# vwxyzjn/cleanrl

Measured on NVIDIA H100. Metric: env steps/sec (SPS) PPO Breakout num_envs=1024, higher is better.
Workload: dtype bf16

## Files before the change

### cleanrl_b200/csrc/net_tc.cu

```cuda
#include <cuda.h>
#include <algorithm>
#include "tc_base.cuh"
#include "tc_conv_win.cuh"
#include "tc_conv1_u8.cuh"
#include "tc_gemm_tma.cuh"
#include "tc_wgrad_win.cuh"
#include "tc_reduce.cuh"
#include "tc_aux.cuh"
#include "tc_heads.cuh"
#include "tc_heads_wide.cuh"
#include "tc_lstm.cuh"

namespace b200rl {

struct NatureLayout {
    int A;
    int64_t c1w, c1b, c2w, c2b, c3w, c3b, fcw, fcb, hw, hb, total;
    int64_t w1f, w2f, w2dg, w3f, w3dg, wfcf, wfcdg, w1l, w1sc, packed_total;
    bool wide; int G; int64_t whf, whdg, hbp;
    int64_t wih, whh, bih, bhh, whhp;
    explicit NatureLayout(int A_) : A(A_), wih(-1), whh(-1), bih(-1), bhh(-1), whhp(-1) {
        int64_t o = 0;
        c1w = o; o += 32 * 4 * 8 * 8;  c1b = o; o += 32;
        c2w = o; o += 64 * 32 * 4 * 4; c2b = o; o += 64;
        c3w = o; o += 64 * 64 * 3 * 3; c3b = o; o += 64;
        fcw = o; o += 512 * 3136;      fcb = o; o += 512;
        hw = o;  o += (int64_t)(A + 1) * 512;
        hb = o;  o += A + 1;
        total = o;
        int64_t q = 0;
        w1f = q; q += 32 * 256;
        w2f = q; q += 64 * 512;
        w2dg = q; q += 4 * 32 * 256;
        w3f = q; q += 64 * 576;
        w3dg = q; q += 64 * 576;
        wfcf = q; q += 512 * 3136;
        wfcdg = q; q += 3136 * 512;
        w1l = q; q += 64 * 256 / 2;
        w1sc = q; q += 64 * 2;
        wide = A + 1 > kMaxHeads;
        G = wide ? (int)ceil_div(A + 1, kWideHeadPad) * kWideHeadPad : 0;
        whf = whdg = hbp = 0;
        if (wide) {
            whf = q; q += (int64_t)G * 512;
            whdg = q; q += (int64_t)G * 512;
            hbp = q; q += (int64_t)G * 2;
        }
        packed_total = q;
    }
    struct Lstm {};
    NatureLayout(int A_, Lstm) : A(A_) {
        int64_t o = 0;
        c1w = o; o += 32 * 8 * 8;      c1b = o; o += 32;
        c2w = o; o += 64 * 32 * 4 * 4; c2b = o; o += 64;
        c3w = o; o += 64 * 64 * 3 * 3; c3b = o; o += 64;
        fcw = o; o += 512 * 3136;      fcb = o; o += 512;
        wih = o; o += 512 * 512;       whh = o; o += 512 * 128;
        bih = o; o += 512;             bhh = o; o += 512;
        hw = o;  o += (int64_t)(A + 1) * 128;
        hb = o;  o += A + 1;
        total = o;
        int64_t q = 0;
        w1f = q; q += 32 * 64;
        w2f = q; q += 64 * 512;
        w2dg = q; q += 4 * 32 * 256;
        w3f = q; q += 64 * 576;
        w3dg = q; q += 64 * 576;
        wfcf = q; q += 512 * 3136;
        wfcdg = q; q += 3136 * 512;
        w1l = w1sc = -1;
        wide = true; G = 512;
        whf = q; q += 512 * 512;
        whdg = q; q += 512 * 512;
        hbp = q; q += 512 * 2;
        whhp = q; q += 512 * 128;
        packed_total = q;
    }
};

struct NatureActs {
    int64_t x0, act1, act2, act3, hid, dhid, dact3a, dact3b, dact2a, dact2b, dact1, m1, m2, m3, m4, total;
    explicit NatureActs(int64_t n, bool with_x0 = true) {
        int64_t o = 0;
        x0 = o; if (with_x0) o += n * 28224;
        act1 = o; o += n * 12800;
        act2 = o; o += n * 5184;
        act3 = o; o += n * 3136;
        hid = o;  o += n * 512;
        dhid = o; o += n * 512;
        dact3a = o; o += n * 5184;
        dact3b = o; o += n * 7744;
        dact2a = o; o += n * 6400;
        dact2b = o; o += n * 7744;
        dact1 = o; o += n * 14112;
        auto pad8 = [](int64_t v) { return (v + 7) & ~int64_t(7); };
        m1 = o; o += pad8(n * 100 * 4 * 2);
        m2 = o; o += pad8(n * 81 * 2 * 2);
        m3 = o; o += pad8(n * 49 * 2 * 2);
        m4 = o; o += pad8(n * 16 * 2);
        total = o;
    }
};

static void gemm_rowmajor(KGemmParams& p, const bf16* x, int64_t n, int nchunks) {
    memset(&p, 0, sizeof(p));
    p.scale = 1.f;
    p.A = x; p.M = n; p.nchunks = nchunks;
}


static void win_defaults(WinParams& p) { memset(&p, 0, sizeof(p)); p.scale = 1.f; }
static int round8(int v) { return (v + 7) & ~7; }
static void win_conv1(WinParams& p, const bf16* x0, const int64_t* rows, int64_t n) {
    p.A = x0; p.rows = rows; p.n = (int)n; p.G = 441; p.Wp = 21; p.M = n * 441;
    p.tpi_shift = 2;
    p.n_images = rows ? (int64_t)1 << 24 : n;
    p.ntaps = 4; p.shift[0] = 0; p.shift[1] = 1; p.shift[2] = 21; p.shift[3] = 22; p.WR = round8(128 + 22);
}
static void win_conv2(WinParams& p, const bf16* act1, int64_t n) {
    p.A = act1; p.n = (int)n; p.G = 100; p.Wp = 10; p.M = n * 100;
    p.ntaps = 4; p.shift[0] = 0; p.shift[1] = 1; p.shift[2] = 10; p.shift[3] = 11; p.WR = round8(128 + 11);
}
static void win_conv3(WinParams& p, const bf16* act2, int64_t n) {
    p.A = act2; p.n = (int)n; p.G = 81; p.Wp = 9; p.M = n * 81;
    p.ntaps = 9; for (int ky = 0; ky < 3; ++ky) for (int kx = 0; kx < 3; ++kx) p.shift[ky * 3 + kx] = ky * 9 + kx;
    p.WR = round8(128 + 20);
}
static void wgw_defaults(WGradWinParams& w) { memset(&w, 0, sizeof(w)); }

static const int kC1Ctas = 264, kC2Ctas = 132, kC3Ctas = 132;
static WPlan conv1_wgrad_plan(int64_t n, bool u8) {
    return u8 ? wgrad_plan(n * 512, kC2Ctas, 512) : wgrad_plan(n * 512, kC1Ctas, 128);
}
static WPlan conv2_wgrad_plan(int64_t n) { return wgrad_plan(n * 100, kC2Ctas, 128); }
static WPlan conv3_wgrad_plan(int64_t n) { return wgrad_plan(n * 81, kC3Ctas, 128); }

static size_t wgrad_win_bytes(int splits, int nslots) { return (size_t)splits * nslots * 64 * 64 * sizeof(float); }
static size_t wgrad_win_bias_bytes(int splits) { return (size_t)splits * 64 * sizeof(float); }
static int launch_wgrad_win(const WGradWinParams& p, int ctas, cudaStream_t s, const char* what) {
    const size_t smem = (size_t)kWgradWinStages * ((size_t)p.WRX * 128 * p.cpr + 128 * 128) + 4096 + 1024;
    static SmemAttrCache attr;
    if (int rc0 = attr.ensure(tc_wgrad_win, smem, what)) return rc0;
    CUtensorMap tmX, tmY;
    memset(&tmX, 0, sizeof(tmX)); memset(&tmY, 0, sizeof(tmY));
    const int use_tma = p.tpi_shift ? 0 : 1;
    if (p.rows_per_cta % 128 != 0) return fail(B200RL_ERR_INVALID_ARGUMENT, "%s: rows per CTA must be a multiple of 128", what);
    if (ctas < 1 || (int64_t)(ctas - 1) * p.rows_per_cta >= p.M)
        return fail(B200RL_ERR_INVALID_ARGUMENT, "%s: every row split must own at least one row", what);
    int rc;
    if (use_tma) {
        if (p.rows || p.ldy != 64 || p.ncolsY != 64)
            return fail(B200RL_ERR_INVALID_ARGUMENT, "%s: linear-grid mode needs contiguous rows and 64-channel dY", what);
        if ((rc = make_tmap_2d(&tmX, p.X, p.M, (int64_t)p.cpr * 64, p.WRX, what))) return rc;
        if ((rc = make_tmap_2d(&tmY, p.Y, p.M, 64, 128, what))) return rc;
    } else {
        if ((128 << p.tpi_shift) < p.G) return fail(B200RL_ERR_INVALID_ARGUMENT, "%s: steps per image too small", what);
        if ((rc = make_tmap_3d(&tmX, p.X, p.n_images, p.G, (int64_t)p.cpr * 64, p.WRX, what))) return rc;
    }
    const dim3 grid((unsigned)ceil_div(p.nslots / 2, kWgradWinTilesPerCta), ctas);
    tc_wgrad_win<<<grid, kWgradWinThreads, smem, s>>>(tmX, tmY, p, use_tma);
    return check_launch(what);
}

}

using namespace b200rl;

namespace b200rl {
static bool head_ok(int A) { return A >= 1 && A < kMaxWideHeads; }
static size_t wide_dhead_bytes(int64_t n, const NatureLayout& L) { return ((size_t)n * L.G * 2 + 255) & ~(size_t)255; }
static size_t wide_small_bytes(int64_t n, const NatureLayout& L, int A1) {
    return wide_dhead_bytes(n, L) + colsum_f32_ws(n, A1);
}

static int trunk_fwd(const NatureLayout& L, const NatureActs& Q, const float* params, const bf16* P, bf16* act, int64_t n,
                     cudaStream_t s) {
    int rc;
    KGemmParams p;
    WinParams wp;
    win_defaults(wp); win_conv2(wp, act + Q.act1, n);
    wp.Bw = P + L.w2f; wp.N = 64; wp.vH = 9; wp.vW = 9; wp.out_mode = WOUT_DENSE; wp.out = act + Q.act2;
    wp.bias = params + L.c2b; wp.relu = 1; wp.mask_out = reinterpret_cast<uint32_t*>(act + Q.m2);
    { ProfScope ps(s, "conv2_fwd", 2.0 * n * 81 * 64 * 512, (double)n * ((12800 + 5184) * 2 + 648));
      if ((rc = launch_conv_win_t<128, 2, 2, 4>(wp, s, "naturecnn/conv2"))) return rc; }
    win_defaults(wp); win_conv3(wp, act + Q.act2, n);
    wp.Bw = P + L.w3f; wp.N = 64; wp.vH = 7; wp.vW = 7; wp.out_mode = WOUT_DENSE; wp.out = act + Q.act3;
    wp.bias = params + L.c3b; wp.relu = 1; wp.mask_out = reinterpret_cast<uint32_t*>(act + Q.m3);
    { ProfScope ps(s, "conv3_fwd", 2.0 * n * 49 * 64 * 576, (double)n * ((5184 + 3136) * 2 + 392));
      if ((rc = launch_conv_win_t<128, 1, 4, 9>(wp, s, "naturecnn/conv3"))) return rc; }
    gemm_rowmajor(p, act + Q.act3, n, 49);
    p.Bw = P + L.wfcf; p.N = 512; p.out = act + Q.hid; p.ldo = 512; p.bias = params + L.fcb; p.relu = 1;
    p.mask_out = reinterpret_cast<uint32_t*>(act + Q.m4);
    { ProfScope ps(s, "fc_fwd", 2.0 * n * 512 * 3136, (double)n * (3136 + 512) * 2 + 512.0 * 3136 * 2);
      if (n <= 8192) { if ((rc = launch_gemm_tma<64, 6>(p, s, "naturecnn/fc"))) return rc; }
      else if ((rc = launch_gemm_tma<128, 4>(p, s, "naturecnn/fc"))) return rc; }
    return B200RL_OK;
}

static int trunk_bwd(const NatureLayout& L, const NatureActs& Q, const bf16* P, bf16* act, float* grads, int64_t n,
                     float* wsbig, float* wssmall, void* tail_ready_event, bool dact1_fused, cudaStream_t s) {
    int rc;
    KGemmParams p;
    {
        int splits;
        { ProfScope ps(s, "fc_wgrad", 2.0 * n * 512 * 3136, (double)n * (3136 + 512) * 2 + 512.0 * 3136 * 4);
          if ((splits = launch_wgrad_tma(act + Q.dhid, 512, act + Q.act3, 3136, n, wsbig, s, "naturecnn/fc_wgrad")) < 0) return splits; }
        { ProfScope ps(s, "wgrad_fold_bias", 0, 0);
          note_launches(1); tc_fold_fc<<<(unsigned)ceil_div((int64_t)512 * 3136, 256), 256, 0, s>>>(wsbig, splits, 512, 13 * 256, 512, 3136, 64, 49, 1.f, grads + L.fcw);
          if ((rc = colsum(act + Q.dhid, n, 512, 512, wssmall, grads + L.fcb, s))) return rc; }
        if (tail_ready_event) {
            cudaError_t e = cudaEventRecord(reinterpret_cast<cudaEvent_t>(tail_ready_event), s);
            if (e != cudaSuccess) return fail(B200RL_ERR_CUDA, "naturecnn_backward: cudaEventRecord: %s", cudaGetErrorString(e));
        }
        gemm_rowmajor(p, act + Q.dhid, n, 8);
        p.Bw = P + L.wfcdg; p.N = 3136; p.out = act + Q.dact3a; p.out2 = act + Q.dact3b; p.dual_dact3 = 1;
        p.ldo = 3136; p.mask_bits = reinterpret_cast<const uint32_t*>(act + Q.m3);
        { ProfScope ps(s, "fc_dgrad", 2.0 * n * 512 * 3136, (double)n * ((3136 + 512) * 2 + 392) + 512.0 * 3136 * 2);
          if ((rc = launch_gemm_tma<128, 4>(p, s, "naturecnn/fc_dgrad"))) return rc; }
    }
    WGradWinParams gw;
    WinParams wp;
    FoldWin fw;
    {
        wgw_defaults(gw);
        gw.X = act + Q.act2; gw.M = n * 81; gw.n = (int)n; gw.G = 81; gw.cpr = 1; gw.nslots = 10; gw.WRX = round8(128 + 20);
        for (int t = 0; t < 9; ++t) gw.shift[t] = (t / 3) * 9 + (t % 3);
        const int st[10] = {0, 1, 2, 3, 4, 5, 6, 7, 7, 8};
        for (int k = 0; k < 10; ++k) { gw.slot_tap[k] = st[k]; gw.slot_cc[k] = 0; }
        gw.Y = act + Q.dact3a; gw.ldy = 64; gw.ncolsY = 64;
        const WPlan pl = conv3_wgrad_plan(n);
        gw.rows_per_cta = pl.rows_per_cta; gw.ws = wsbig; gw.wsb = wssmall;
        { ProfScope ps(s, "conv3_wgrad", 2.0 * n * 49 * 64 * 576, (double)n * (5184 + 5184) * 2);
          if ((rc = launch_wgrad_win(gw, pl.splits, s, "naturecnn/conv3_wgrad"))) return rc; }
        memset(&fw, 0, sizeof(fw));
        fw.layer = 3; fw.S = pl.splits; fw.nslots = 10; fw.Cout = 64; fw.scale = 1.f; fw.bscale = 1.f;
        for (int k = 0; k < 10; ++k) { fw.slot_tap[k] = st[k]; fw.slot_skip[k] = (k == 8); }
        { ProfScope ps(s, "wgrad_fold_bias", 0, 0);
          fw.wsb = wssmall; fw.db = grads + L.c3b;
          tc_fold_win<<<(unsigned)ceil_div(640 * 64 + 64, 32), 256, 0, s>>>(wsbig, fw, grads + L.c3w);
          if ((rc = check_launch("naturecnn/conv3_fold"))) return rc; }
        win_defaults(wp);
        wp.A = act + Q.dact3b; wp.n = (int)n; wp.G = 121; wp.Wp = 11; wp.M = n * 121; wp.ntaps = 9;
        for (int ky = 0; ky < 3; ++ky) for (int kx = 0; kx < 3; ++kx) wp.shift[ky * 3 + kx] = (2 - ky) * 11 + (2 - kx);
        wp.WR = round8(128 + 24);
        wp.Bw = P + L.w3dg; wp.N = 64; wp.vH = 9; wp.vW = 9; wp.out_mode = WOUT_DACT2;
        wp.out = act + Q.dact2a; wp.out2 = act + Q.dact2b; wp.mask_bits = reinterpret_cast<const uint32_t*>(act + Q.m2);
        { ProfScope ps(s, "conv3_dgrad", 2.0 * n * 81 * 64 * 576, (double)n * ((7744 + 6400 + 7744) * 2 + 648));
          if ((rc = launch_conv_win_t<128, 1, 4, 9>(wp, s, "naturecnn/conv3_dgrad"))) return rc; }
    }
    {
        wgw_defaults(gw);
        gw.X = act + Q.act1; gw.M = n * 100; gw.n = (int)n; gw.G = 100; gw.cpr = 2; gw.nslots = 8; gw.WRX = round8(128 + 11);
        gw.shift[0] = 0; gw.shift[1] = 1; gw.shift[2] = 10; gw.shift[3] = 11;
        for (int k = 0; k < 8; ++k) { gw.slot_tap[k] = k >> 1; gw.slot_cc[k] = k & 1; }
        gw.Y = act + Q.dact2a; gw.ldy = 64; gw.ncolsY = 64;
        const WPlan pl = conv2_wgrad_plan(n);
        gw.rows_per_cta = pl.rows_per_cta; gw.ws = wsbig; gw.wsb = wssmall;
        { ProfScope ps(s, "conv2_wgrad", 2.0 * n * 81 * 64 * 512, (double)n * (12800 + 6400) * 2);
          if ((rc = launch_wgrad_win(gw, pl.splits, s, "naturecnn/conv2_wgrad"))) return rc; }
        memset(&fw, 0, sizeof(fw));
        fw.layer = 2; fw.S = pl.splits; fw.nslots = 8; fw.Cout = 64; fw.scale = 1.f; fw.bscale = 1.f;
        for (int k = 0; k < 8; ++k) { fw.slot_tap[k] = k >> 1; fw.slot_cc[k] = k & 1; }
        { ProfScope ps(s, "wgrad_fold_bias", 0, 0);
          fw.wsb = wssmall; fw.db = grads + L.c2b;
          tc_fold_win<<<(unsigned)ceil_div(512 * 64 + 64, 32), 256, 0, s>>>(wsbig, fw, grads + L.c2w);
          if ((rc = check_launch("naturecnn/conv2_fold"))) return rc; }
        if (dact1_fused) return B200RL_OK;
        win_defaults(wp);
        wp.A = act + Q.dact2b; wp.n = (int)n; wp.G = 121; wp.Wp = 11; wp.M = n * 121; wp.ntaps = 4;
        for (int a = 0; a < 2; ++a) for (int b = 0; b < 2; ++b) wp.shift[a * 2 + b] = (1 - a) * 11 + (1 - b);
        wp.WR = round8(128 + 12);
        wp.Bw = P + L.w2dg; wp.N = 128; wp.vH = 10; wp.vW = 10; wp.out_mode = WOUT_DACT1;
        wp.out = act + Q.dact1; wp.mask_bits = reinterpret_cast<const uint32_t*>(act + Q.m1);
        { ProfScope ps(s, "conv2_dgrad", 2.0 * n * 400 * 32 * 256, (double)n * ((7744 + 14112) * 2 + 1600));
          if ((rc = launch_conv_win<128, 1, 4, 4>(wp, s, "naturecnn/conv2_dgrad"))) return rc; }
    }
    return B200RL_OK;
}
static size_t trunk_big_bytes(int64_t n) {
    return std::max({wgrad_tma_bytes(n, 512, 3136), wgrad_win_bytes(conv3_wgrad_plan(n).splits, 10),
                     wgrad_win_bytes(conv2_wgrad_plan(n).splits, 8)});
}
static size_t trunk_small_bytes(int64_t n) {
    return std::max({colsum_ws(n, 512), wgrad_win_bias_bytes(conv3_wgrad_plan(n).splits),
                     wgrad_win_bias_bytes(conv2_wgrad_plan(n).splits)});
}

static int wide_head_fwd(const NatureLayout& L, const bf16* P, const bf16* hid, int64_t n, int A1, float* out, cudaStream_t s) {
    KGemmParams p;
    gemm_rowmajor(p, hid, n, 8);
    p.Bw = P + L.whf; p.N = L.G; p.bias = reinterpret_cast<const float*>(P + L.hbp);
    p.out_f32 = out; p.ldo = A1; p.ncols_f32 = A1;
    return launch_gemm_tma<128, 4>(p, s, "wide_heads");
}

static int wide_head_bwd(const NatureLayout& L, const bf16* P, const float* dhead, int64_t n, int A1, const bf16* hid, bf16* dhid,
                         const uint32_t* hid_bits, float* dW, float* db, float* wsbig, float* wssmall, cudaStream_t s) {
    int rc;
    KGemmParams p;
    bf16* dh16 = reinterpret_cast<bf16*>(wssmall);
    float* dbpart = reinterpret_cast<float*>(reinterpret_cast<char*>(wssmall) + wide_dhead_bytes(n, L));
    int cb = (int)ceil_div(n * L.G, 256); if (cb > num_sms() * 8) cb = num_sms() * 8;
    tc_head_dhead_bf16<<<cb, 256, 0, s>>>(dhead, n, A1, L.G, dh16);
    if ((rc = check_launch("wide_heads_dhead"))) return rc;
    if ((rc = colsum_f32(dhead, n, A1, dbpart, db, s))) return rc;
    const int splits = launch_wgrad_tma(dh16, L.G, hid, 512, n, wsbig, s, "wide_heads_wgrad");
    if (splits < 0) return splits;
    tc_fold_fc<<<(unsigned)ceil_div((int64_t)A1 * 512, 256), 256, 0, s>>>(wsbig, splits, L.G, 512, A1, 512, 512, 1, 1.f, dW);
    if ((rc = check_launch("wide_heads_wgrad"))) return rc;
    gemm_rowmajor(p, dh16, n, L.G / 64);
    p.Bw = P + L.whdg; p.N = 512; p.out = dhid; p.ldo = 512;
    p.mask_bits = hid_bits;
    if (n <= 8192) { if ((rc = launch_gemm_tma<64, 6>(p, s, "wide_heads_dgrad"))) return rc; }
    else if ((rc = launch_gemm_tma<128, 4>(p, s, "wide_heads_dgrad"))) return rc;
    return B200RL_OK;
}
}

extern "C" int64_t b200rl_naturecnn_param_count(int A) { return A >= 1 ? NatureLayout(A).total : -1; }
extern "C" int64_t b200rl_naturecnn_grad_tail_offset(int A) { return A >= 1 ? NatureLayout(A).fcw : -1; }
extern "C" size_t b200rl_naturecnn_bf16_packed_bytes(int A) { return head_ok(A) ? (size_t)NatureLayout(A).packed_total * 2 : 0; }
extern "C" size_t b200rl_naturecnn_bf16_acts_bytes(int64_t n, int obs_format) {
    return n >= 0 ? (size_t)NatureActs(n, obs_format == B200RL_OBS_U8_NCHW).total * 2 + 256 : 0;
}

extern "C" int b200rl_frames_to_s2d_bf16(const uint8_t* obs, const int64_t* rows, int64_t n, void* out, void* stream) {
    B200RL_REQUIRE(n >= 0, "frames_to_s2d: negative n");
    if (n == 0) return B200RL_OK;
    B200RL_REQUIRE(obs && out, "frames_to_s2d: null pointer");
    B200RL_REQUIRE(aligned(obs, 4) && aligned(out, 16), "frames_to_s2d: misaligned buffer");
    cudaStream_t s = (cudaStream_t)stream;
    ProfScope ps(s, "frames_to_s2d", 0, (double)n * 28224 * 3);
    tc_frames_to_s2d<<<(unsigned)ceil_div(n * 1764, 256), 256, 0, s>>>(obs, rows, n, reinterpret_cast<bf16*>(out));
    return check_launch("frames_to_s2d");
}

extern "C" int b200rl_frames_to_s2d_u8(const uint8_t* obs, const int64_t* rows, int64_t n, uint8_t* out_rm, uint8_t* out_cm, void* stream) {
    B200RL_REQUIRE(n >= 0, "frames_to_s2d_u8: negative n");
    if (n == 0) return B200RL_OK;
    B200RL_REQUIRE(obs && out_rm && out_cm, "frames_to_s2d_u8: null pointer");
    B200RL_REQUIRE(aligned(obs, 16) && aligned(out_rm, 16) && aligned(out_cm, 16), "frames_to_s2d_u8: misaligned buffer");
    B200RL_REQUIRE(n <= (int64_t)1 << 28, "frames_to_s2d_u8: n too large");
    cudaStream_t s = (cudaStream_t)stream;
    ProfScope ps(s, "frames_to_s2d", 0, (double)n * (28224 + 28224 + 28672));
    tc_frames_to_s2d_u8<<<(unsigned)(n * 4), 256, 0, s>>>(obs, rows, n, out_rm, out_cm);
    return check_launch("frames_to_s2d_u8");
}

static size_t naturecnn_big_bytes(int64_t n, const NatureLayout& L) {
    return std::max({trunk_big_bytes(n), L.wide ? wgrad_tma_bytes(n, L.G, 512) : 0,
                     wgrad_win_bytes(conv1_wgrad_plan(n, false).splits, 4), wgrad_win_bytes(conv1_wgrad_plan(n, true).splits, 4)});
}

extern "C" size_t b200rl_naturecnn_bf16_workspace_bytes(int64_t n, int A) {
    if (n < 1 || !head_ok(A)) return 0;
    const NatureLayout L(A);
    const size_t small = std::max({trunk_small_bytes(n), L.wide ? wide_small_bytes(n, L, A + 1) : heads_partial_bytes(n, A + 1, 512),
                                   wgrad_win_bias_bytes(conv1_wgrad_plan(n, false).splits),
                                   wgrad_win_bias_bytes(conv1_wgrad_plan(n, true).splits)});
    return naturecnn_big_bytes(n, L) + small + 512;
}

extern "C" int b200rl_naturecnn_bf16_pack(const float* params, int A, void* packed, void* stream) {
    B200RL_REQUIRE(params && packed && head_ok(A), "naturecnn_pack: bad arguments (A must be in [1,%d])", kMaxWideHeads - 1);
    B200RL_REQUIRE(aligned(packed, 16), "naturecnn_pack: packed buffer must be 16-B aligned");
    const NatureLayout L(A);
    bf16* P = reinterpret_cast<bf16*>(packed);
    cudaStream_t s = (cudaStream_t)stream;
    ProfScope ps(s, "pack_weights", 0, (double)L.total * 4 + (double)L.packed_total * 2);
    tc_pack_conv1_s2d<<<32, 256, 0, s>>>(params + L.c1w, P + L.w1f);
    tc_pack_conv1_i8<<<32, 256, 0, s>>>(params + L.c1w, reinterpret_cast<int8_t*>(P + L.w1l), reinterpret_cast<float*>(P + L.w1sc));
    tc_pack_conv2_cells<<<128, 256, 0, s>>>(params + L.c2w, P + L.w2f);
    tc_pack_conv_s2_classes<<<(unsigned)ceil_div(32768, 256), 256, 0, s>>>(params + L.c2w, 64, 32, P + L.w2dg);
    tc_pack_conv<<<(unsigned)ceil_div(36864, 256), 256, 0, s>>>(params + L.c3w, 64, 64, 3, 3, 0, P + L.w3f, P + L.w3dg);
    tc_pack_fc<<<dim3(512 / 8, 49 / 7), 256, 0, s>>>(params + L.fcw, 512, 49, P + L.wfcf, P + L.wfcdg);
    if (L.wide) {
        tc_pack_head_wide<<<(unsigned)ceil_div((int64_t)L.G * 512, 256), 256, 0, s>>>(params + L.hw, params + L.hb, A + 1, L.G,
                                                                                    P + L.whf, P + L.whdg, reinterpret_cast<float*>(P + L.hbp));
        return check_launch("naturecnn_pack", 7);
    }
    return check_launch("naturecnn_pack", 6);
}

extern "C" int b200rl_naturecnn_bf16_forward(const void* obs, int obs_format, const int64_t* rows, int64_t n, int A,
                                             const float* params, const void* packed, void* acts,
                                             float* head_out, void* stream) {
    B200RL_REQUIRE(n >= 0, "naturecnn_forward: negative n");
    if (n == 0) return B200RL_OK;
    B200RL_REQUIRE(obs && params && packed && acts && head_out, "naturecnn_forward: null pointer");
    B200RL_REQUIRE(head_ok(A), "naturecnn_forward: A=%d outside [1,%d]", A, kMaxWideHeads - 1);
    B200RL_REQUIRE(obs_format == B200RL_OBS_U8_NCHW || obs_format == B200RL_OBS_S2D_BF16 || obs_format == B200RL_OBS_S2D_U8,
                   "naturecnn_forward: bad obs_format %d", obs_format);
    B200RL_REQUIRE(aligned(obs, 16) && aligned(acts, 16) && aligned(packed, 16), "naturecnn_forward: misaligned buffer");
    B200RL_REQUIRE(n <= (int64_t)1 << 22, "naturecnn_forward: n too large");
    const NatureLayout L(A);
    const NatureActs Q(n, obs_format == B200RL_OBS_U8_NCHW);
    const bf16* P = reinterpret_cast<const bf16*>(packed);
    bf16* act = reinterpret_cast<bf16*>(acts);
    cudaStream_t s = (cudaStream_t)stream;
    int rc;
    WinParams wp;
    const bf16* x0 = reinterpret_cast<const bf16*>(obs);
    const int64_t* x0rows = rows;
    if (obs_format == B200RL_OBS_U8_NCHW) {
        if ((rc = b200rl_frames_to_s2d_bf16(reinterpret_cast<const uint8_t*>(obs), rows, n, act + Q.x0, stream))) return rc;
        x0 = act + Q.x0; x0rows = nullptr;
    }
    if (obs_format == B200RL_OBS_S2D_U8) {
        Conv1U8Params cp;
        memset(&cp, 0, sizeof(cp));
        cp.rows = rows; cp.n = (int)n; cp.n_images = rows ? (int64_t)1 << 24 : n;
        cp.limbs = reinterpret_cast<const int8_t*>(P + L.w1l); cp.sc = reinterpret_cast<const float*>(P + L.w1sc);
        cp.bias = params + L.c1b; cp.out = act + Q.act1; cp.mask_out = reinterpret_cast<uint32_t*>(act + Q.m1);
        ProfScope ps(s, "conv1_fwd", 2.0 * n * 400 * 32 * 256, (double)n * (28224 + 12800 * 2 + 1600));
        if ((rc = launch_conv1_i8(cp, obs, s, "naturecnn/conv1_i8"))) return rc;
    } else {
    win_defaults(wp); win_conv1(wp, x0, x0rows, n);
    wp.Bw = P + L.w1f; wp.N = 32; wp.vH = 20; wp.vW = 20; wp.out_mode = WOUT_S2D2; wp.out = act + Q.act1;
    wp.bias = params + L.c1b; wp.scale = 1.0f / 255.0f; wp.relu = 1; wp.mask_out = reinterpret_cast<uint32_t*>(act + Q.m1);
    { ProfScope ps(s, "conv1_fwd", 2.0 * n * 400 * 32 * 256, (double)n * ((28224 + 12800) * 2 + 1600));
      if ((rc = launch_conv_win<32, 1, 9, 4>(wp, s, "naturecnn/conv1"))) return rc; }
    }
    if ((rc = trunk_fwd(L, Q, params, P, act, n, s))) return rc;
    if (L.wide) {
        ProfScope ps(s, "heads_fwd", 2.0 * n * 512 * (A + 1), (double)n * (1024 + 4 * (A + 1)) + (double)L.G * 1024);
        return wide_head_fwd(L, P, act + Q.hid, n, A + 1, head_out, s);
    }
    ProfScope ps(s, "heads_fwd", 2.0 * n * 512 * (A + 1), (double)n * (1024 + 4 * (A + 1)));
    return heads_fwd<512>(act + Q.hid, params + L.hw, params + L.hb, n, A + 1, head_out, s, "naturecnn/heads");
}

extern "C" int b200rl_naturecnn_bf16_backward(const void* obs, const void* obs_aux, int obs_format, const int64_t* rows, int64_t n, int A,
                                              const float* params, const void* packed, void* acts,
                                              const float* dhead, float* grads,
                                              void* workspace, size_t workspace_bytes, void* tail_ready_event, void* stream) {
    B200RL_REQUIRE(n >= 1, "naturecnn_backward: n must be >= 1");
    B200RL_REQUIRE(obs && params && packed && acts && dhead && grads && workspace, "naturecnn_backward: null pointer");
    B200RL_REQUIRE(head_ok(A), "naturecnn_backward: A=%d outside [1,%d]", A, kMaxWideHeads - 1);
    B200RL_REQUIRE(aligned(workspace, 16), "naturecnn_backward: workspace misaligned");
    const size_t need = b200rl_naturecnn_bf16_workspace_bytes(n, A);
    if (workspace_bytes < need) return fail(B200RL_ERR_WORKSPACE, "naturecnn_backward: workspace %zu < %zu", workspace_bytes, need);
    B200RL_REQUIRE(obs_format == B200RL_OBS_U8_NCHW || obs_format == B200RL_OBS_S2D_BF16 || obs_format == B200RL_OBS_S2D_U8,
                   "naturecnn_backward: bad obs_format %d", obs_format);
    B200RL_REQUIRE(obs_format != B200RL_OBS_S2D_U8 || (obs_aux && aligned(obs_aux, 16)), "naturecnn_backward: the uint8 rollout needs obs_aux");
    const NatureLayout L(A);
    const NatureActs Q(n, obs_format == B200RL_OBS_U8_NCHW);
    const bf16* P = reinterpret_cast<const bf16*>(packed);
    bf16* act = reinterpret_cast<bf16*>(acts);
    cudaStream_t s = (cudaStream_t)stream;
    const bf16* x0 = obs_format == B200RL_OBS_U8_NCHW ? act + Q.x0 : reinterpret_cast<const bf16*>(obs);
    const int64_t* x0rows = obs_format == B200RL_OBS_U8_NCHW ? nullptr : rows;
    const size_t big = (naturecnn_big_bytes(n, L) + 255) & ~(size_t)255;
    float* wsbig = reinterpret_cast<float*>(workspace);
    float* wssmall = reinterpret_cast<float*>(reinterpret_cast<char*>(workspace) + big);
    int rc;
    const int A1 = A + 1;
    if (L.wide) {
        ProfScope ps(s, "heads_bwd", 4.0 * n * 512 * A1, (double)n * (2048 + 64 + 8 * A1));
        if ((rc = wide_head_bwd(L, P, dhead, n, A1, act + Q.hid, act + Q.dhid, reinterpret_cast<const uint32_t*>(act + Q.m4),
                                grads + L.hw, grads + L.hb, wsbig, wssmall, s))) return rc;
    } else
    {
        ProfScope ps(s, "heads_bwd", 4.0 * n * 512 * A1, (double)n * (2048 + 64 + 8 * A1));
        if ((rc = heads_bwd_weight<512>(dhead, act + Q.hid, n, A1, wssmall, grads + L.hw, grads + L.hb, s, "naturecnn/heads_bwd"))) return rc;
        if ((rc = heads_bwd_data<512>(dhead, params + L.hw, reinterpret_cast<const uint8_t*>(act + Q.m4), n, A1, act + Q.dhid, s,
                                      "naturecnn/heads_bwd"))) return rc;
    }
    if ((rc = trunk_bwd(L, Q, P, act, grads, n, wsbig, wssmall, tail_ready_event, obs_format == B200RL_OBS_S2D_U8, s))) return rc;
    const bool u8 = obs_format == B200RL_OBS_S2D_U8;
    const WPlan pl = conv1_wgrad_plan(n, u8);
    if (u8) {
        Conv21BwdU8Params cw;
        memset(&cw, 0, sizeof(cw));
        cw.rows = rows; cw.n = (int)n; cw.rows_per_cta = pl.rows_per_cta; cw.ws = wsbig; cw.wsb = wssmall;
        cw.w2dg = P + L.w2dg; cw.m1 = reinterpret_cast<const uint32_t*>(act + Q.m1);
        { ProfScope ps(s, "conv21_bwd", 2.0 * 2.0 * n * 400 * 32 * 256, (double)n * (7744 * 2 + 1600 + 28672 + 14112 * 2));
          if ((rc = launch_conv21_bwd_u8(cw, obs_aux, rows ? (int64_t)1 << 24 : n, act + Q.dact2b, act + Q.dact1, pl.splits, s,
                                         "naturecnn/conv21_bwd_u8"))) return rc; }
    } else {
        WGradWinParams gw;
        wgw_defaults(gw);
        gw.X = x0; gw.rows = x0rows; gw.M = n * 512; gw.n = (int)n; gw.G = 441; gw.cpr = 1; gw.nslots = 4; gw.WRX = round8(128 + 22);
        gw.tpi_shift = 2; gw.n_images = x0rows ? (int64_t)1 << 24 : n;
        gw.shift[0] = 0; gw.shift[1] = 1; gw.shift[2] = 21; gw.shift[3] = 22;
        for (int k = 0; k < 4; ++k) { gw.slot_tap[k] = k; gw.slot_cc[k] = 0; }
        gw.Y = act + Q.dact1; gw.ldy = 32; gw.ncolsY = 32;
        gw.rows_per_cta = pl.rows_per_cta; gw.ws = wsbig; gw.wsb = wssmall;
        { ProfScope ps(s, "conv1_wgrad", 2.0 * n * 400 * 32 * 256, (double)n * (28224 + 14112) * 2);
          if ((rc = launch_wgrad_win(gw, pl.splits, s, "naturecnn/conv1_wgrad"))) return rc; }
    }
    FoldWin fw;
    memset(&fw, 0, sizeof(fw));
    fw.layer = 1; fw.S = pl.splits; fw.nslots = 4; fw.Cout = 32;
    fw.scale = u8 ? 1.0f / 255.0f / kDact1Scale : 1.0f / 255.0f;
    fw.bscale = u8 ? 1.0f / kDact1Scale : 1.f;
    for (int k = 0; k < 4; ++k) fw.slot_tap[k] = k;
    { ProfScope ps(s, "wgrad_fold_bias", 0, 0);
      fw.wsb = wssmall; fw.db = grads + L.c1b;
      tc_fold_win<<<(unsigned)ceil_div(256 * 32 + 32, 32), 256, 0, s>>>(wsbig, fw, grads + L.c1w);
      if ((rc = check_launch("naturecnn/conv1_fold"))) return rc; }
    return B200RL_OK;
}

namespace b200rl {
constexpr int64_t kLstmMaxRows = (int64_t)1 << 17;

struct LstmActs {
    NatureActs T;
    int64_t gx, hseq, hm, save, cm, dgates, total;
    explicit LstmActs(int64_t M) : T(M, false) {
        int64_t o = (T.total * 2 + 255) & ~int64_t(255);
        auto take = [&](int64_t bytes) { const int64_t r = o; o += (bytes + 255) & ~int64_t(255); return r; };
        gx = take(M * 512 * 4);
        hseq = take(M * 128 * 2);
        hm = take(M * 128 * 2);
        save = take(M * 640 * 4);
        cm = take(M * 128 * 4);
        dgates = take(M * 512 * 4);
        total = o;
    }
};

static bool lstm_heads_ok(int A) { return A >= 1 && A + 1 <= lstm::kMaxA1; }
static bool lstm_sizes_ok(int64_t S, int64_t n) { return S >= 1 && n >= 1 && S <= kLstmMaxRows && n <= kLstmMaxRows && S * n <= kLstmMaxRows; }

struct C1Plan { int64_t per_cta; int ctas; };
static C1Plan lstm_conv1_plan(int64_t M) {
    C1Plan c;
    const int64_t want = M < kC1Ctas ? M : kC1Ctas;
    c.per_cta = ceil_div(M, want);
    c.ctas = (int)ceil_div(M, c.per_cta);
    return c;
}
static size_t lstm_big_bytes(int64_t M, const NatureLayout& L) {
    const size_t a = std::max({wgrad_tma_bytes(M, L.G, 512), wgrad_tma_bytes(M, 512, 128), trunk_big_bytes(M),
                               (size_t)lstm_conv1_plan(M).ctas * 32 * 64 * 4});
    return (a + 255) & ~(size_t)255;
}
static size_t lstm_small_bytes(int64_t M, const NatureLayout& L) {
    return std::max({heads_partial_bytes(M, L.A + 1, 128), wide_small_bytes(M, L, 512), trunk_small_bytes(M),
                     (size_t)lstm_conv1_plan(M).ctas * 32 * 4});
}
}

extern "C" int64_t b200rl_lstm_agent_param_count(int A) { return A >= 1 ? NatureLayout(A, NatureLayout::Lstm{}).total : -1; }
extern "C" size_t b200rl_lstm_agent_bf16_packed_bytes(int A) {
    return lstm_heads_ok(A) ? (size_t)NatureLayout(A, NatureLayout::Lstm{}).packed_total * 2 : 0;
}
extern "C" size_t b200rl_lstm_agent_bf16_acts_bytes(int64_t S, int64_t n) {
    return lstm_sizes_ok(S, n) ? (size_t)LstmActs(S * n).total : 0;
}
extern "C" int b200rl_lstm_agent_bf16_acts_layout(int64_t S, int64_t n, int64_t* offsets) {
    B200RL_REQUIRE(offsets, "lstm_acts_layout: null pointer");
    B200RL_REQUIRE(lstm_sizes_ok(S, n), "lstm_acts_layout: S=%lld n=%lld out of range", (long long)S, (long long)n);
    const LstmActs Q(S * n);
    const int64_t v[B200RL_LSTM_ACTS_TENSORS] = {Q.T.act1 * 2, Q.T.m1 * 2, Q.T.act2 * 2, Q.T.act3 * 2, Q.T.hid * 2, Q.T.m4 * 2,
                                                 Q.gx, Q.hseq, Q.hm, Q.save, Q.cm, Q.dgates, Q.T.dhid * 2};
    for (int k = 0; k < B200RL_LSTM_ACTS_TENSORS; ++k) offsets[k] = v[k];
    return B200RL_OK;
}
extern "C" size_t b200rl_lstm_agent_bf16_workspace_bytes(int64_t S, int64_t n, int A) {
    if (!lstm_sizes_ok(S, n) || !lstm_heads_ok(A)) return 0;
    const NatureLayout L(A, NatureLayout::Lstm{});
    return lstm_big_bytes(S * n, L) + lstm_small_bytes(S * n, L) + 512;
}

extern "C" int b200rl_lstm_agent_bf16_pack(const float* params, int A, void* packed, void* stream) {
    B200RL_REQUIRE(params && packed, "lstm_pack: null pointer");
    B200RL_REQUIRE(lstm_heads_ok(A), "lstm_pack: A=%d outside [1,%d]", A, lstm::kMaxA1 - 1);
    B200RL_REQUIRE(aligned(params, 16) && aligned(packed, 16), "lstm_pack: misaligned buffer");
    const NatureLayout L(A, NatureLayout::Lstm{});
    bf16* P = reinterpret_cast<bf16*>(packed);
    cudaStream_t s = (cudaStream_t)stream;
    ProfScope ps(s, "pack_weights", 0, (double)L.total * 4 + (double)L.packed_total * 2);
    lstm::lstm_pack_conv1<<<8, 256, 0, s>>>(params + L.c1w, P + L.w1f);
    tc_pack_conv2_cells<<<128, 256, 0, s>>>(params + L.c2w, P + L.w2f);
    tc_pack_conv_s2_classes<<<(unsigned)ceil_div(32768, 256), 256, 0, s>>>(params + L.c2w, 64, 32, P + L.w2dg);
    tc_pack_conv<<<(unsigned)ceil_div(36864, 256), 256, 0, s>>>(params + L.c3w, 64, 64, 3, 3, 0, P + L.w3f, P + L.w3dg);
    tc_pack_fc<<<dim3(512 / 8, 49 / 7), 256, 0, s>>>(params + L.fcw, 512, 49, P + L.wfcf, P + L.wfcdg);
    tc_pack_head_wide<<<(unsigned)ceil_div((int64_t)L.G * 512, 256), 256, 0, s>>>(params + L.wih, params + L.bih, 512, L.G,
                                                                                P + L.whf, P + L.whdg, reinterpret_cast<float*>(P + L.hbp));
    tc_head_dhead_bf16<<<256, 256, 0, s>>>(params + L.whh, 512, 128, 128, P + L.whhp);
    return check_launch("lstm_pack", 7);
}

extern "C" int b200rl_lstm_agent_bf16_forward(const uint8_t* obs, const int64_t* rows, int64_t S, int64_t n, int A,
                                              const float* params, const void* packed, const float* h0, const float* c0,
                                              const float* done, void* acts, float* head_out, float* h_out, float* c_out,
                                              void* stream) {
    B200RL_REQUIRE(obs && params && packed && h0 && c0 && done && acts && head_out && h_out && c_out, "lstm_forward: null pointer");
    B200RL_REQUIRE(lstm_heads_ok(A), "lstm_forward: A=%d outside [1,%d]", A, lstm::kMaxA1 - 1);
    B200RL_REQUIRE(lstm_sizes_ok(S, n), "lstm_forward: S=%lld n=%lld (S*n at most %lld)", (long long)S, (long long)n,
                   (long long)kLstmMaxRows);
    B200RL_REQUIRE(aligned(obs, 16) && aligned(rows, 8) && aligned(params, 16) && aligned(packed, 16) && aligned(acts, 256) &&
                   aligned(h0, 16) && aligned(c0, 16) && aligned(done, 4) && aligned(head_out, 4) && aligned(h_out, 16) &&
                   aligned(c_out, 16), "lstm_forward: misaligned buffer");
    const int64_t M = S * n;
    const NatureLayout L(A, NatureLayout::Lstm{});
    const LstmActs Q(M);
    const bf16* P = reinterpret_cast<const bf16*>(packed);
    uint8_t* ab = reinterpret_cast<uint8_t*>(acts);
    bf16* act = reinterpret_cast<bf16*>(acts);
    cudaStream_t s = (cudaStream_t)stream;
    int rc;
    {
        lstm::Conv1P cp;
        cp.obs = obs; cp.rows = rows; cp.n = M; cp.w = P + L.w1f; cp.bias = params + L.c1b; cp.out = act + Q.T.act1;
        cp.mask_out = reinterpret_cast<uint32_t*>(act + Q.T.m1);
        ProfScope ps(s, "conv1_fwd", 2.0 * M * 400 * 32 * 64, (double)M * (7056 + 12800 * 2 + 1600));
        const int64_t grid = M < (int64_t)num_sms() * 8 ? M : (int64_t)num_sms() * 8;
        lstm::lstm_conv1_fwd<<<(unsigned)grid, lstm::kThreads, lstm::conv1_fwd_smem(), s>>>(cp);
        if ((rc = check_launch("lstm/conv1"))) return rc;
    }
    if ((rc = trunk_fwd(L, Q.T, params, P, act, M, s))) return rc;
    float* gx = reinterpret_cast<float*>(ab + Q.gx);
    { ProfScope ps(s, "lstm_ih_fwd", 2.0 * M * 512 * 512, (double)M * (1024 + 2048) + 512.0 * 1024);
      if ((rc = wide_head_fwd(L, P, act + Q.T.hid, M, 512, gx, s))) return rc; }
    {
        lstm::RecFwdP rp;
        rp.S = (int)S; rp.n = n; rp.whh = P + L.whhp; rp.bhh = params + L.bhh; rp.gx = gx; rp.done = done; rp.h0 = h0; rp.c0 = c0;
        rp.hseq = reinterpret_cast<bf16*>(ab + Q.hseq); rp.hm = reinterpret_cast<bf16*>(ab + Q.hm);
        rp.save = reinterpret_cast<float*>(ab + Q.save); rp.cm = reinterpret_cast<float*>(ab + Q.cm);
        rp.h_out = h_out; rp.c_out = c_out;
        static SmemAttrCache attr;
        if ((rc = attr.ensure(lstm::lstm_rec_fwd, lstm::rec_fwd_smem(), "lstm/recurrence"))) return rc;
        ProfScope ps(s, "lstm_rec_fwd", 2.0 * M * 512 * 128, (double)M * (2048 + 4 + 512 + 3840) + 131072.0);
        lstm::lstm_rec_fwd<<<(unsigned)ceil_div(n, lstm::kRows), lstm::kThreads, lstm::rec_fwd_smem(), s>>>(rp);
        if ((rc = check_launch("lstm/recurrence"))) return rc;
    }
    ProfScope ps(s, "heads_fwd", 2.0 * M * 128 * (A + 1), (double)M * (256 + 4 * (A + 1)));
    return heads_fwd<128>(reinterpret_cast<const bf16*>(ab + Q.hseq), params + L.hw, params + L.hb, M, A + 1, head_out, s, "lstm/heads");
}

extern "C" int b200rl_lstm_agent_bf16_backward(const uint8_t* obs, const int64_t* rows, int64_t S, int64_t n, int A,
                                               const float* params, const void* packed, const float* done, void* acts,
                                               const float* dhead, float* grads, void* workspace, size_t workspace_bytes,
                                               void* stream) {
    B200RL_REQUIRE(obs && params && packed && done && acts && dhead && grads && workspace, "lstm_backward: null pointer");
    B200RL_REQUIRE(lstm_heads_ok(A), "lstm_backward: A=%d outside [1,%d]", A, lstm::kMaxA1 - 1);
    B200RL_REQUIRE(lstm_sizes_ok(S, n), "lstm_backward: S=%lld n=%lld (S*n at most %lld)", (long long)S, (long long)n,
                   (long long)kLstmMaxRows);
    B200RL_REQUIRE(aligned(obs, 16) && aligned(rows, 8) && aligned(params, 16) && aligned(packed, 16) && aligned(acts, 256) &&
                   aligned(done, 4) && aligned(dhead, 4) && aligned(grads, 16) && aligned(workspace, 256),
                   "lstm_backward: misaligned buffer");
    const size_t need = b200rl_lstm_agent_bf16_workspace_bytes(S, n, A);
    if (workspace_bytes < need) return fail(B200RL_ERR_WORKSPACE, "lstm_backward: workspace %zu < %zu", workspace_bytes, need);
    const int64_t M = S * n;
    const int A1 = A + 1;
    const NatureLayout L(A, NatureLayout::Lstm{});
    const LstmActs Q(M);
    const bf16* P = reinterpret_cast<const bf16*>(packed);
    uint8_t* ab = reinterpret_cast<uint8_t*>(acts);
    bf16* act = reinterpret_cast<bf16*>(acts);
    cudaStream_t s = (cudaStream_t)stream;
    float* wsbig = reinterpret_cast<float*>(workspace);
    float* wssmall = reinterpret_cast<float*>(reinterpret_cast<char*>(workspace) + lstm_big_bytes(M, L));
    const bf16* hseq = reinterpret_cast<const bf16*>(ab + Q.hseq);
    float* dgates = reinterpret_cast<float*>(ab + Q.dgates);
    int rc;
    {
        ProfScope ps(s, "heads_bwd", 2.0 * M * 128 * A1, (double)M * (256 + 4 * A1));
        if ((rc = heads_bwd_weight<128>(dhead, hseq, M, A1, wssmall, grads + L.hw, grads + L.hb, s, "lstm/heads_bwd"))) return rc;
    }
    {
        lstm::RecBwdP bp;
        bp.S = (int)S; bp.n = n; bp.A1 = A1; bp.whh = P + L.whhp; bp.wh = params + L.hw; bp.dhead = dhead; bp.done = done;
        bp.save = reinterpret_cast<const float*>(ab + Q.save); bp.cm = reinterpret_cast<const float*>(ab + Q.cm);
        bp.dgates = dgates;
        static SmemAttrCache attr;
        if ((rc = attr.ensure(lstm::lstm_rec_bwd, lstm::rec_bwd_smem(), "lstm/recurrence_bwd"))) return rc;
        ProfScope ps(s, "lstm_rec_bwd", 2.0 * M * 512 * 128 + 2.0 * M * 128 * A1, (double)M * (4 * A1 + 3072 + 2048));
        lstm::lstm_rec_bwd<<<(unsigned)ceil_div(n, lstm::kRows), lstm::kThreads, lstm::rec_bwd_smem(), s>>>(bp);
        if ((rc = check_launch("lstm/recurrence_bwd"))) return rc;
    }
    {
        ProfScope ps(s, "lstm_ih_bwd", 4.0 * M * 512 * 512, (double)M * (2048 + 1024 * 3 + 64));
        if ((rc = wide_head_bwd(L, P, dgates, M, 512, act + Q.T.hid, act + Q.T.dhid, reinterpret_cast<const uint32_t*>(act + Q.T.m4),
                                grads + L.wih, grads + L.bih, wsbig, wssmall, s))) return rc;
    }
    {
        ProfScope ps(s, "lstm_hh_wgrad", 2.0 * M * 512 * 128, (double)M * (1024 + 256) + 512.0 * 128 * 4);
        const int splits = launch_wgrad_tma(wssmall, 512, ab + Q.hm, 128, M, wsbig, s, "lstm/hh_wgrad");
        if (splits < 0) return splits;
        tc_fold_fc<<<(unsigned)ceil_div((int64_t)512 * 128, 256), 256, 0, s>>>(wsbig, splits, 512, 64 * kFcWgradYChunks, 512, 128,
                                                                            128, 1, 1.f, grads + L.whh);
        if ((rc = check_launch("lstm/hh_wgrad"))) return rc;
        const cudaError_t e = cudaMemcpyAsync(grads + L.bhh, grads + L.bih, 512 * sizeof(float), cudaMemcpyDeviceToDevice, s);
        if (e != cudaSuccess) return fail(B200RL_ERR_CUDA, "lstm_backward: bias copy: %s", cudaGetErrorString(e));
    }
    if ((rc = trunk_bwd(L, Q.T, P, act, grads, M, wsbig, wssmall, nullptr, false, s))) return rc;
    {
        const C1Plan pl = lstm_conv1_plan(M);
        lstm::Conv1WgradP wp;
        wp.obs = obs; wp.rows = rows; wp.n = M; wp.dy = act + Q.T.dact1; wp.imgs_per_cta = pl.per_cta; wp.ws = wsbig; wp.wsb = wssmall;
        static SmemAttrCache attr;
        if ((rc = attr.ensure(lstm::lstm_conv1_wgrad, lstm::conv1_wgrad_smem(), "lstm/conv1_wgrad"))) return rc;
        ProfScope ps(s, "conv1_wgrad", 2.0 * M * 400 * 32 * 64, (double)M * (7056 + 14112 * 2));
        lstm::lstm_conv1_wgrad<<<pl.ctas, lstm::kThreads, lstm::conv1_wgrad_smem(), s>>>(wp);
        lstm::lstm_conv1_fold<<<(unsigned)ceil_div(32 * 64 + 32, 256), 256, 0, s>>>(wsbig, wssmall, pl.ctas, grads + L.c1w, grads + L.c1b);
        if ((rc = check_launch("lstm/conv1_wgrad", 2))) return rc;
    }
    return B200RL_OK;
}
```

### cleanrl_b200/csrc/tc_conv1_u8.cuh

```cuda
#pragma once
#include "tc_base.cuh"
#include <cuda_fp16.h>
#include "tc_conv_win.cuh"

namespace b200rl {
using namespace tc;

__device__ __forceinline__ uint64_t desc_kmajor_sw64(uint32_t smem_addr) {
    return (uint64_t)((smem_addr & 0x3FFFFu) >> 4) | (1ull << 16) | (32ull << 32) | kDescSwizzle64;
}
__device__ __forceinline__ uint64_t desc_mnmajor_sw64(uint32_t smem_addr, uint32_t lbo) {
    return (uint64_t)((smem_addr & 0x3FFFFu) >> 4) | ((uint64_t)((lbo >> 4) & 0x3FFF) << 16) | (32ull << 32) | kDescSwizzle64;
}
__device__ __forceinline__ uint32_t img64_off(int r, int c) { return (uint32_t)(r * 64 + ((c ^ ((r >> 1) & 3)) << 4)); }
__global__ void __launch_bounds__(256) tc_frames_to_s2d_u8(const uint8_t* __restrict__ obs, const int64_t* __restrict__ rows, int64_t n,
                                                           uint8_t* __restrict__ out_rm, uint8_t* __restrict__ out_cm) {
    __shared__ __align__(16) uint8_t plane[7056];
    const int64_t i = blockIdx.x >> 2;
    const int c = blockIdx.x & 3;
    const int64_t img = rows ? rows[i] : i;
    const int4* src = reinterpret_cast<const int4*>(obs + img * 28224 + c * 7056);
    for (int t = threadIdx.x; t < 441; t += 256) reinterpret_cast<int4*>(plane)[t] = __ldg(src + t);
    __syncthreads();
    for (int pos = threadIdx.x; pos < 441; pos += 256) {
        const int Y = pos / 21, X = pos - Y * 21;
        const uint8_t* p = plane + (Y * 4) * 84 + X * 4;
        int4 v;
        v.x = *reinterpret_cast<const int*>(p); v.y = *reinterpret_cast<const int*>(p + 84);
        v.z = *reinterpret_cast<const int*>(p + 168); v.w = *reinterpret_cast<const int*>(p + 252);
        *reinterpret_cast<int4*>(out_rm + (i * 441 + pos) * 64 + c * 16) = v;
    }
    for (int t = threadIdx.x; t < 16 * 112; t += 256) {
        const int ch = t / 112, q = t - ch * 112;
        const int sy = ch >> 2, sx = ch & 3;
        uint32_t w = 0;
#pragma unroll
        for (int e = 0; e < 4; ++e) {
            const int pos = q * 4 + e;
            if (pos < 441) {
                const int Y = pos / 21, X = pos - Y * 21;
                w |= (uint32_t)plane[(Y * 4 + sy) * 84 + X * 4 + sx] << (8 * e);
            }
        }
        *reinterpret_cast<uint32_t*>(out_cm + (i * 64 + c * 16 + ch) * 448 + q * 4) = w;
    }
}

__global__ void __launch_bounds__(256) tc_pack_conv1_i8(const float* __restrict__ w, int8_t* __restrict__ limbs, float* __restrict__ sc) {
    __shared__ float red[32];
    const int co = blockIdx.x, idx = threadIdx.x;
    const float v = w[co * 256 + idx];
    float m = fabsf(v);
#pragma unroll
    for (int o = 16; o > 0; o >>= 1) m = fmaxf(m, __shfl_xor_sync(0xffffffffu, m, o));
    if ((idx & 31) == 0) red[idx >> 5] = m;
    __syncthreads();
    float mx = red[0];
#pragma unroll
    for (int k = 1; k < 8; ++k) mx = fmaxf(mx, red[k]);
    const float s = mx > 0.f ? mx * (128.0f / 127.0f) : 1.0f;
    const float u = v / s * 128.0f;
    float l1 = rintf(u);
    l1 = fminf(fmaxf(l1, -127.f), 127.f);
    float l2 = rintf((u - l1) * 128.0f);
    l2 = fminf(fmaxf(l2, -127.f), 127.f);
    const int kx = idx & 7, ky = (idx >> 3) & 7, c = idx >> 6;
    const int a = ky >> 2, sy = ky & 3, b = kx >> 2, sx = kx & 3;
    const int k = (a * 2 + b) * 64 + c * 16 + sy * 4 + sx;
    limbs[co * 256 + k] = (int8_t)l1;
    limbs[(32 + co) * 256 + k] = (int8_t)l2;
    if (idx == 0) {
        sc[co] = s / 128.0f / 255.0f;
        sc[32 + co] = s / 16384.0f / 255.0f;
    }
}

struct Conv1U8Params {
    const int64_t* rows;
    int n;
    int64_t n_images;
    const int8_t* limbs;
    const float* sc;
    const float* bias;
    bf16* out;
    uint32_t* mask_out;
};

constexpr int kConv1I8Threads = 384;
template <int STAGES>
__global__ void __launch_bounds__(kConv1I8Threads, 1) tc_conv1_i8(const __grid_constant__ CUtensorMap tmA, const Conv1U8Params p, int total_tiles) {
    constexpr int BN = 64, WR = 144, NTAPS = 4;
    constexpr int STAGE_BYTES = WR * 128;
    constexpr int B_CHUNK = BN * 64;
    extern __shared__ uint8_t smem_raw[];
    __shared__ uint64_t full_bar[STAGES], empty_bar[STAGES];
    __shared__ __align__(16) float s_sc[32], s_bias[32];
    uint8_t* smem = reinterpret_cast<uint8_t*>((reinterpret_cast<uintptr_t>(smem_raw) + 1023) & ~uintptr_t(1023));
    const int tid = threadIdx.x, warp = tid >> 5;
    uint8_t* sW = smem;
    uint8_t* sRing = smem + NTAPS * B_CHUNK;

    if (tid == 0) {
        for (int s = 0; s < STAGES; ++s) { mbar_init(&full_bar[s], 1); mbar_init(&empty_bar[s], 8); }
        fence_barrier_init();
        tma_prefetch_desc(&tmA);
    }
    for (int idx = tid; idx < NTAPS * BN * 4; idx += blockDim.x) {
        const int c16 = idx & 3;
        const int t = (idx >> 2) & 3;
        const int r = idx >> 4;
        *reinterpret_cast<int4*>(sW + t * B_CHUNK + img64_off(r, c16)) = ldg16(p.limbs + r * 256 + t * 64 + c16 * 16);
    }
    if (tid < 32) { s_sc[tid] = p.sc[32 + tid]; s_bias[tid] = p.bias[tid]; }
    fence_proxy_async_smem();
    __syncthreads();
    const int tile_begin = (int)(((int64_t)total_tiles * blockIdx.x) / gridDim.x);
    const int tile_end = (int)(((int64_t)total_tiles * (blockIdx.x + 1)) / gridDim.x);

    if (warp == 0) {
        if (tid == 0) {
            uint32_t q = 0;
            int z_next = 0;
            if (tile_begin < tile_end) {
                const int img = tile_begin >> 1;
                z_next = p.rows ? (int)__ldg(p.rows + img) : img;
            }
            for (int tile = tile_begin; tile < tile_end; ++tile, ++q) {
                const uint32_t s = q % STAGES;
                const int z = z_next;
                if (tile + 1 < tile_end) {
                    const int img = (tile + 1) >> 1;
                    z_next = p.rows ? (int)__ldg(p.rows + img) : img;
                }
                if (q >= (uint32_t)STAGES) mbar_wait(&empty_bar[s], ((q / STAGES) - 1) & 1);
                mbar_arrive_expect_tx(&full_bar[s], (uint32_t)STAGE_BYTES);
                tma_load_3d(smem_u32(sRing + (size_t)s * STAGE_BYTES), &tmA, 0, (tile & 1) * 128, z, &full_bar[s]);
            }
        }
    } else if (warp >= 4) {
        const int wg = (warp - 4) >> 2, wt = tid & 127, lane = tid & 31, qd = lane & 3;
        const uint32_t w_base = smem_u32(sW);
        constexpr int off[4] = {0, 1, 21, 22};
        int acc[2][32];
#pragma unroll
        for (int e = 0; e < 2; ++e)
#pragma unroll
            for (int c = 0; c < 32; ++c) acc[e][c] = 0;
        for (int tile = tile_begin; tile < tile_end; ++tile) {
            const uint32_t q = (uint32_t)(tile - tile_begin), s = q % STAGES;
            mbar_wait(&full_bar[s], (q / STAGES) & 1);
            wgmma_fence();
            const uint32_t win = smem_u32(sRing + (size_t)s * STAGE_BYTES) + (uint32_t)(wg * 64 * 128);
#pragma unroll
            for (int e = 0; e < 2; ++e) {
#pragma unroll
                for (int t = 0; t < NTAPS; ++t) {
                    const int po = e + off[t];
                    const uint64_t a = desc_kmajor(win + (uint32_t)((po >> 1) * 128 + (po & 1) * 64));
                    const uint64_t b = desc_kmajor_sw64(w_base + (uint32_t)(t * B_CHUNK));
#pragma unroll
                    for (int kk = 0; kk < 2; ++kk) wgmma_u8s8_n64(acc[e], a + 2 * kk, b + 2 * kk, (t | kk) != 0 ? 1u : 0u);
                }
            }
            wgmma_commit();
            wgmma_wait<0>();
            wgmma_fence_operands(acc[0]);
            wgmma_fence_operands(acc[1]);
            if (lane == 0) mbar_arrive(&empty_bar[s]);
            const int i = tile >> 1;
#pragma unroll
            for (int e = 0; e < 2; ++e) {
#pragma unroll
                for (int hr = 0; hr < 2; ++hr) {
                    const int lrow = wg * 64 + ((wt >> 5) << 4) + (lane >> 2) + 8 * hr;
                    const int rem = 2 * (((tile & 1) << 7) + lrow) + e;
                    const int Y = (rem * 3121) >> 16, X = rem - Y * 21;
                    const bool valid = rem < 441 && Y < 20 && X < 20;
                    const int64_t cell = ((int64_t)i * 10 + (Y >> 1)) * 10 + (X >> 1);
                    const int cls = (Y & 1) * 2 + (X & 1);
                    uint32_t bits = 0u, pk[4];
#pragma unroll
                    for (int j = 0; j < 4; ++j) {
                        const int co = 8 * j + 2 * qd;
                        const float f0 = fmaf((float)(acc[e][4 * j + 2 * hr] * 128 + acc[e][4 * (j + 4) + 2 * hr]), s_sc[co], s_bias[co]);
                        const float f1 = fmaf((float)(acc[e][4 * j + 2 * hr + 1] * 128 + acc[e][4 * (j + 4) + 2 * hr + 1]), s_sc[co + 1],
                                              s_bias[co + 1]);
                        bits |= (f0 > 0.f ? 1u : 0u) << co;
                        bits |= (f1 > 0.f ? 1u : 0u) << (co + 1);
                        pk[j] = pack_bf16x2_relu(f0, f1);
                    }
                    bits |= __shfl_xor_sync(0xffffffffu, bits, 1);
                    bits |= __shfl_xor_sync(0xffffffffu, bits, 2);
                    if (valid) {
                        if (qd == 0) p.mask_out[cell * 4 + cls] = bits;
                        uint32_t* dst = reinterpret_cast<uint32_t*>(reinterpret_cast<uint8_t*>(p.out) + (cell * 4 + cls) * 64);
#pragma unroll
                        for (int j = 0; j < 4; ++j) dst[4 * j + qd] = pk[j];
                    }
                }
            }
        }
    }
}

struct Conv21BwdU8Params {
    const int64_t* rows;
    int n;
    int64_t rows_per_cta;
    const bf16* w2dg;
    const uint32_t* m1;
    float* ws;
    float* wsb;
};
constexpr int kC1WXStages = 6, kC21WinStages = 2;
constexpr int kC1WBlock = 64 * 128, kC1WYBytes = 128 * 64, kC1WYPadRows = 24, kC1WYPad = kC1WYPadRows * 64;
constexpr int kC1WShift = 21;
constexpr int kC21WinRows = 140, kC21WinBytes = 18 * 1024;
constexpr int kC21W2Bytes = 4 * 128 * 128;
constexpr int kC21ImgBytes = kC1WYPad + 4 * kC1WYBytes;
constexpr float kDact1Scale = 4096.0f;

__device__ __forceinline__ uint32_t prmt(uint32_t a, uint32_t b, uint32_t sel) {
    uint32_t d;
    asm("prmt.b32 %0, %1, %2, %3;" : "=r"(d) : "r"(a), "r"(b), "r"(sel));
    return d;
}
constexpr float kU8Bias = 1024.0f;


__device__ __forceinline__ uint32_t pair_f16_biased(const uint32_t (&w)[5], int j, bool up, uint32_t sel) {
    const uint32_t lo = up ? w[j + 1] : w[j];
    const uint32_t hi = up ? w[j + 2] : w[j + 1];
    return prmt(prmt(lo, hi, sel), 0x64646464u, 0x5140u);
}
__device__ __forceinline__ uint4 lds128(uint32_t addr) {
    uint4 v;
    asm volatile("ld.shared.v4.u32 {%0, %1, %2, %3}, [%4];" : "=r"(v.x), "=r"(v.y), "=r"(v.z), "=r"(v.w) : "r"(addr) : "memory");
    return v;
}
__device__ __forceinline__ uint32_t pack_f16x2_sat(float lo, float hi) {
    uint32_t d;
    asm("cvt.rn.satfinite.f16x2.f32 %0, %1, %2;" : "=r"(d) : "f"(hi), "f"(lo));
    return d;
}

__device__ __forceinline__ void sts32(uint32_t addr, uint32_t v) { asm volatile("st.shared.u32 [%0], %1;" ::"r"(addr), "r"(v) : "memory"); }
__device__ __forceinline__ void tma_store_3d(const void* tmap, uint32_t smem_src, int x, int y, int z) {
    asm volatile("cp.async.bulk.tensor.3d.global.shared::cta.bulk_group [%0, {%1, %2, %3}], [%4];"
                 ::"l"(reinterpret_cast<uint64_t>(tmap)), "r"(x), "r"(y), "r"(z), "r"(smem_src) : "memory");
}
__device__ __forceinline__ void bulk_commit() { asm volatile("cp.async.bulk.commit_group;" ::: "memory"); }
template <int N> __device__ __forceinline__ void bulk_wait_read() { asm volatile("cp.async.bulk.wait_group.read %0;" ::"n"(N) : "memory"); }
template <int N> __device__ __forceinline__ void bulk_wait() { asm volatile("cp.async.bulk.wait_group %0;" ::"n"(N) : "memory"); }

template <int R> __device__ __forceinline__ void setmaxnreg_dec() { asm volatile("setmaxnreg.dec.sync.aligned.u32 %0;" ::"n"(R)); }
template <int R> __device__ __forceinline__ void setmaxnreg_inc() { asm volatile("setmaxnreg.inc.sync.aligned.u32 %0;" ::"n"(R)); }
constexpr int kC1WRegsProducer = 40, kC21RegsDgrad = 128, kC1WRegsMma = 168;
static_assert(128 * kC1WRegsProducer + 128 * kC21RegsDgrad + 256 * kC1WRegsMma <= 65536, "register budgets exceed the SM");

constexpr int kC1WThreads = 512;
__global__ void __launch_bounds__(kC1WThreads, 1) tc_conv21_bwd_u8(const __grid_constant__ CUtensorMap tmX, const __grid_constant__ CUtensorMap tmWin,
                                                                 const __grid_constant__ CUtensorMap tmY, const Conv21BwdU8Params p) {
    constexpr int XS = kC1WXStages, WS = kC21WinStages;
    extern __shared__ uint8_t smem_raw[];
    __shared__ uint64_t xfull[XS], xempty[XS], wfull[WS], wempty[WS], yfull[2], yempty[2];
    __shared__ float sRed[32 * 32], sBias[32];
    uint8_t* smem = reinterpret_cast<uint8_t*>((reinterpret_cast<uintptr_t>(smem_raw) + 1023) & ~uintptr_t(1023));
    uint8_t* sW2 = smem;
    uint8_t* sWin = sW2 + kC21W2Bytes;
    uint8_t* sX = sWin + (size_t)WS * kC21WinBytes;
    uint8_t* sImg = sX + (size_t)XS * kC1WBlock;
    const int tid = threadIdx.x, warp = tid >> 5, lane = tid & 31;
    if (tid == 0) {
        for (int s = 0; s < XS; ++s) { mbar_init(&xfull[s], 1); mbar_init(&xempty[s], 12); }
        for (int s = 0; s < WS; ++s) { mbar_init(&wfull[s], 1); mbar_init(&wempty[s], 4); }
        for (int s = 0; s < 2; ++s) { mbar_init(&yfull[s], 1); mbar_init(&yempty[s], 8); }
        fence_barrier_init();
        tma_prefetch_desc(&tmX);
        tma_prefetch_desc(&tmWin);
        tma_prefetch_desc(&tmY);
    }
    for (int idx = tid; idx < 4 * 128 * 8; idx += blockDim.x) {
        const int c16 = idx & 7, r = (idx >> 3) & 127, t = idx >> 10;
        *reinterpret_cast<int4*>(sW2 + t * (128 * 128) + img_off(r, c16)) = ldg16(p.w2dg + r * 256 + t * 64 + c16 * 8);
    }
    for (int idx = tid; idx < 2 * kC21ImgBytes / 16; idx += blockDim.x) reinterpret_cast<int4*>(sImg)[idx] = make_int4(0, 0, 0, 0);
    fence_proxy_async_smem();
    __syncthreads();
    const int64_t M = (int64_t)p.n * 512;
    const int64_t m_begin = (int64_t)blockIdx.x * p.rows_per_cta;
    int64_t m_end = m_begin + p.rows_per_cta;
    if (m_end > M) m_end = M;
    const int nsteps = m_end > m_begin ? (int)((m_end - m_begin) >> 7) : 0;
    const int nimg = nsteps >> 2;
    const int64_t g0 = m_begin >> 7;
    const int img0 = (int)(m_begin >> 9);

    if (warp < 4) {
        setmaxnreg_dec<kC1WRegsProducer>();
        if (warp == 0 && lane == 0 && nsteps > 0) {
            auto image_of = [&](int64_t g) -> int {
                int64_t img = g >> 2;
                if (img >= p.n) img = p.n - 1;
                return p.rows ? (int)__ldg(p.rows + img) : (int)img;
            };
            int z = image_of(g0), z_next = image_of(g0 + 4);
            for (int k = 0; k <= nsteps; ++k) {
                const int64_t g = g0 + k;
                if (k > 0 && (g & 3) == 0) { z = z_next; z_next = image_of(g + 4); }
                const int xs = k % XS;
                if (k >= XS) mbar_wait(&xempty[xs], ((k / XS) - 1) & 1);
                mbar_arrive_expect_tx(&xfull[xs], (uint32_t)kC1WBlock);
                tma_load_3d(smem_u32(sX + (size_t)xs * kC1WBlock), &tmX, (int)(g & 3) * 128, 0, z, &xfull[xs]);
            }
        } else if (warp == 1 && lane == 0) {
            for (int j = 0; j < nimg; ++j) {
                const int s = j % WS;
                if (j >= WS) mbar_wait(&wempty[s], ((j / WS) - 1) & 1);
                mbar_arrive_expect_tx(&wfull[s], (uint32_t)(kC21WinRows * 128));
                tma_load_2d(smem_u32(sWin + (size_t)s * kC21WinBytes), &tmWin, 0, (img0 + j) * 121, &wfull[s]);
            }
        }
    } else if (warp < 8) {
        const int wt = tid - 128, lane4 = lane >> 2, qd = lane & 3;
        const uint32_t w_base = smem_u32(sW2);
        const int rq = wt >> 2, c16 = wt & 3;
        float bsum[8];
#pragma unroll
        for (int e = 0; e < 8; ++e) bsum[e] = 0.f;
        for (int j = 0; j < nimg; ++j) {
            const int i = img0 + j, buf = j & 1, s = j % WS;
            const uint32_t img = smem_u32(sImg + (size_t)buf * kC21ImgBytes) + kC1WYPad;
            mbar_wait(&wfull[s], (j / WS) & 1);
            if (j >= 2) mbar_wait(&yempty[buf], ((j >> 1) - 1) & 1);
            if (wt == 0) bulk_wait_read<1>();
            named_bar(1, 128);
#pragma unroll 1
            for (int h2 = 0; h2 < 2; ++h2) {
                float d[64];
                wgmma_fence();
                const uint32_t win = smem_u32(sWin + (size_t)s * kC21WinBytes) + (uint32_t)(h2 * 64 * 128);
                constexpr int shift[4] = {12, 11, 1, 0};
#pragma unroll
                for (int t = 0; t < 4; ++t) {
                    const uint64_t a = desc_kmajor(win + (uint32_t)shift[t] * 128u);
                    const uint64_t b = desc_kmajor(w_base + (uint32_t)(t * 128 * 128));
#pragma unroll
                    for (int kk = 0; kk < 4; ++kk) WgmmaBf16<128, 0, 0>::mma(d, a + 2 * kk, b + 2 * kk, (t | kk) != 0 ? 1u : 0u);
                }
                wgmma_commit();
                int pos[2];
                uint4 mb[2];
#pragma unroll
                for (int hr = 0; hr < 2; ++hr) {
                    const int r = h2 * 64 + ((wt >> 5) << 4) + lane4 + 8 * hr;
                    const int Y = (r * 5958) >> 16, X = r - Y * 11;
                    const bool valid = Y < 10 && X < 10;
                    pos[hr] = valid ? 2 * Y * 21 + 2 * X : -1;
                    mb[hr] = make_uint4(0u, 0u, 0u, 0u);
                    if (valid) {
                        const int4 t = ldg16(p.m1 + ((int64_t)i * 100 + Y * 10 + X) * 4);
                        mb[hr] = make_uint4((uint32_t)t.x, (uint32_t)t.y, (uint32_t)t.z, (uint32_t)t.w);
                    }
                }
                wgmma_wait<0>();
                wgmma_fence_operands(d);
                if (h2 == 1 && lane == 0) mbar_arrive(&wempty[s]);
#pragma unroll
                for (int hr = 0; hr < 2; ++hr) {
                    if (pos[hr] < 0) continue;
                    const uint32_t mw[4] = {mb[hr].x, mb[hr].y, mb[hr].z, mb[hr].w};
#pragma unroll
                    for (int jj = 0; jj < 16; ++jj) {
                        const int g = jj >> 2, c = 8 * (jj & 3) + 2 * qd;
                        float f0 = d[4 * jj + 2 * hr] * kDact1Scale, f1 = d[4 * jj + 2 * hr + 1] * kDact1Scale;
                        if (!((mw[g] >> c) & 1u)) f0 = 0.f;
                        if (!((mw[g] >> (c + 1)) & 1u)) f1 = 0.f;
                        const int q = pos[hr] + (g >> 1) * 21 + (g & 1);
                        sts32(img + img64_off(q, c >> 3) + (uint32_t)((c & 7) * 2), pack_f16x2_sat(f0, f1));
                    }
                }
            }
            fence_proxy_async_smem();
            named_bar(1, 128);
            if (wt == 0) {
                mbar_arrive(&yfull[buf]);
#pragma unroll
                for (int k = 0; k < 4; ++k) tma_store_3d(&tmY, img + (uint32_t)(k * kC1WYBytes), 0, k * 128, i);
                bulk_commit();
            }
#pragma unroll 1
            for (int st = 0; st < 4; ++st) {
#pragma unroll
                for (int ps = 0; ps < 4; ++ps) {
                    const uint4 v = lds128(img + (uint32_t)(st * kC1WYBytes) + img64_off(ps * 32 + rq, c16));
                    const uint32_t w[4] = {v.x, v.y, v.z, v.w};
#pragma unroll
                    for (int e = 0; e < 4; ++e) {
                        const float2 f = __half22float2(*reinterpret_cast<const __half2*>(&w[e]));
                        bsum[2 * e] += f.x;
                        bsum[2 * e + 1] += f.y;
                    }
                }
            }
        }
        if (wt == 0) bulk_wait<0>();
#pragma unroll
        for (int e = 0; e < 8; ++e) sRed[rq * 32 + c16 * 8 + e] = bsum[e];
        named_bar(1, 128);
        if (wt < 32) {
            float t = 0.f;
#pragma unroll
            for (int l = 0; l < 32; ++l) t += sRed[l * 32 + wt];
            p.wsb[(int64_t)blockIdx.x * 64 + wt] = t;
            sBias[wt] = t * kU8Bias;
        }
        named_bar(2, 384);
    } else {
        setmaxnreg_inc<kC1WRegsMma>();
        const int h = (warp - 8) >> 2, wt = tid & 127, qd = lane & 3;
        const int c0 = ((wt >> 5) << 4) + (lane >> 2);
        const bool up = qd >= 2;
        const uint32_t pb = (uint32_t)((2 * qd + h) & 3), psel = pb | ((pb + 1) << 4);
        float d[32];
#pragma unroll
        for (int e = 0; e < 32; ++e) d[e] = 0.f;
        for (int it = 0; it < nsteps; ++it) {
            const int xm = it % XS, xh = (it + 1) % XS, buf = (it >> 2) & 1;
            mbar_wait(&xfull[xm], (it / XS) & 1);
            if (h == 1) mbar_wait(&xfull[xh], ((it + 1) / XS) & 1);
            uint32_t a[8][4];
#pragma unroll
            for (int r = 0; r < 2; ++r) {
                const int c = c0 + 8 * r;
                const uint32_t bm = smem_u32(sX + (size_t)xm * kC1WBlock + c * 128);
                const uint32_t bh = smem_u32(sX + (size_t)xh * kC1WBlock + c * 128);
                const uint32_t sw = (uint32_t)(c & 7);
                uint4 cur = lds128(bm + ((0u ^ sw) << 4));
#pragma unroll
                for (int kk = 0; kk < 8; ++kk) {
                    uint4 nxt = make_uint4(0, 0, 0, 0);
                    if (h == 1) nxt = lds128((kk < 7 ? bm : bh) + ((((uint32_t)(kk + 1) & 7u) ^ sw) << 4));
                    const uint32_t w[5] = {cur.x, cur.y, cur.z, cur.w, nxt.x};
                    a[kk][r] = pair_f16_biased(w, 0, up, psel);
                    a[kk][2 + r] = pair_f16_biased(w, 2, up, psel);
                    if (kk < 7) cur = h == 1 ? nxt : lds128(bm + ((((uint32_t)(kk + 1)) ^ sw) << 4));
                }
            }
            __syncwarp();
            if (lane == 0) {
                mbar_arrive(&xempty[xm]);
                if (h == 1) { mbar_arrive(&xempty[xh]); if (it == 0) mbar_arrive(&xempty[xm]); }
            }
            if ((it & 3) == 0) mbar_wait(&yfull[buf], (it >> 3) & 1);
            wgmma_fence();
            const uint32_t ystep = smem_u32(sImg + (size_t)buf * kC21ImgBytes) + (uint32_t)(kC1WYPad + (it & 3) * kC1WYBytes);
            const uint64_t yd = desc_mnmajor_sw64(ystep - kC1WShift * 64, kC1WShift * 64);
#pragma unroll
            for (int kk = 0; kk < 8; ++kk) wgmma_f16_rs_n64_tb(d, a[kk], yd + 64 * kk, (it | kk) != 0 ? 1u : 0u);
            wgmma_commit();
            wgmma_wait<0>();
            if ((it & 3) == 3 && lane == 0) mbar_arrive(&yempty[buf]);
        }
        wgmma_fence_operands(d);
        named_bar(2, 384);
        float* wsc = p.ws + (int64_t)blockIdx.x * 256 * 64;
#pragma unroll
        for (int b = 0; b < 2; ++b) {
#pragma unroll
            for (int r = 0; r < 2; ++r) {
                float* dst = wsc + (int64_t)((2 * b + h) * 64 + c0 + 8 * r) * 64;
#pragma unroll
                for (int j = 0; j < 4; ++j) {
                    const int co = 8 * j + 2 * qd, e = (b == 0 ? 16 : 0) + 4 * j + 2 * r;
                    *reinterpret_cast<float2*>(dst + co) = make_float2(d[e] - sBias[co], d[e + 1] - sBias[co + 1]);
                }
            }
        }
    }
}

static int launch_conv21_bwd_u8(const Conv21BwdU8Params& p, const void* frames_cm, int64_t n_images, const bf16* dact2b, void* dact1_f16,
                                int ctas, cudaStream_t s, const char* what) {
    const size_t smem = (size_t)kC21W2Bytes + (size_t)kC21WinStages * kC21WinBytes + (size_t)kC1WXStages * kC1WBlock + 2 * (size_t)kC21ImgBytes + 1024;
    int rc;
    if (p.rows_per_cta % 512 != 0) return fail(B200RL_ERR_INVALID_ARGUMENT, "%s: a CTA must own whole images (512 grid rows)", what);
    CUtensorMap tmX, tmWin, tmY;
    memset(&tmX, 0, sizeof(tmX)); memset(&tmWin, 0, sizeof(tmWin)); memset(&tmY, 0, sizeof(tmY));
    if ((rc = make_tmap_3d_u8(&tmX, frames_cm, n_images, 64, 448, 448, 64, 128, what))) return rc;
    if ((rc = make_tmap_2d(&tmWin, dact2b, (int64_t)p.n * 121, 64, kC21WinRows, what))) return rc;
    if ((rc = make_tmap_3d_u8(&tmY, dact1_f16, p.n, 441, 64, 64, 128, 64, what))) return rc;
    static SmemAttrCache attr;
    if ((rc = attr.ensure(tc_conv21_bwd_u8, smem, what))) return rc;
    tc_conv21_bwd_u8<<<ctas, kC1WThreads, smem, s>>>(tmX, tmWin, tmY, p);
    return check_launch(what);
}

constexpr int kConv1I8Stages = 8;
static int launch_conv1_i8(const Conv1U8Params& p, const void* frames_rm, cudaStream_t s, const char* what) {
    constexpr int STAGES = kConv1I8Stages;
    const size_t smem = (size_t)4 * 64 * 64 + (size_t)STAGES * 144 * 128 + 1024;
    const int total = p.n * 2;
    int grid = num_sms();
    if (grid > total) grid = total;
    CUtensorMap tmA;
    memset(&tmA, 0, sizeof(tmA));
    int rc = make_tmap_pairs_u8(&tmA, frames_rm, p.n_images, what);
    if (rc) return rc;
    static SmemAttrCache attr;
    if ((rc = attr.ensure(tc_conv1_i8<STAGES>, smem, what))) return rc;
    tc_conv1_i8<STAGES><<<grid, kConv1I8Threads, smem, s>>>(tmA, p, total);
    return check_launch(what);
}

}
```

### cleanrl_b200/csrc/tc_conv_win.cuh

```cuda
#pragma once
#include "tc_base.cuh"

namespace b200rl {
using namespace tc;

enum { WOUT_DENSE = 0, WOUT_S2D2 = 1, WOUT_DACT2 = 2, WOUT_DACT1 = 3 };
struct WinParams {
    const bf16* A;
    const int64_t* rows;
    int64_t M;
    int n, G, Wp;
    int tpi_shift;
    int64_t n_images;
    int ntaps;
    int shift[16];
    int WR;
    const bf16* Bw;
    int N;
    int vH, vW;
    int out_mode;
    bf16* out;
    bf16* out2;
    const uint32_t* mask_bits;
    uint32_t* mask_out;
    const float* bias;
    float scale;
    int relu;
};

constexpr int kConvWinThreads = 384;
template <int BN>
__host__ __device__ constexpr size_t conv_win_acc_bytes() { return (size_t)128 * (BN + 4) * sizeof(float); }
template <int BN, int CPR, int STAGES, int NTAPS>
__global__ void __launch_bounds__(kConvWinThreads, 1) tc_conv_win(const __grid_constant__ CUtensorMap tmA, const WinParams p,
                                                                  int total_tiles) {
    constexpr int B_CHUNK = BN * 128;
    constexpr int LDA = BN + 4;
    extern __shared__ uint8_t smem_raw[];
    __shared__ uint64_t full_bar[STAGES], empty_bar[STAGES];
    uint8_t* smem = reinterpret_cast<uint8_t*>((reinterpret_cast<uintptr_t>(smem_raw) + 1023) & ~uintptr_t(1023));
    const int tid = threadIdx.x, warp = tid >> 5;
    const int nchunks = p.ntaps * CPR;
    const int K = nchunks * 64;
    const int IMG = p.WR * 128;
    const int STAGE_BYTES = IMG * CPR;
    uint8_t* sW = smem;
    uint8_t* sRing = smem + (size_t)nchunks * B_CHUNK;
    float* sAcc = reinterpret_cast<float*>(sRing + (size_t)STAGES * STAGE_BYTES);

    if (tid == 0) {
        for (int s = 0; s < STAGES; ++s) { mbar_init(&full_bar[s], 1); mbar_init(&empty_bar[s], 8); }
        fence_barrier_init();
        tma_prefetch_desc(&tmA);
    }
    for (int idx = tid; idx < nchunks * BN * 8; idx += blockDim.x) {
        const int c16 = idx & 7;
        int t = idx >> 3;
        const int r = t % BN; const int j = t / BN;
        int4 v = make_int4(0, 0, 0, 0);
        if (r < p.N) v = ldg16(p.Bw + (int64_t)r * K + j * 64 + c16 * 8);
        *reinterpret_cast<int4*>(sW + (size_t)j * B_CHUNK + img_off(r, c16)) = v;
    }
    fence_proxy_async_smem();
    __syncthreads();
    const int tile_begin = (int)(((int64_t)total_tiles * blockIdx.x) / gridDim.x);
    const int tile_end = (int)(((int64_t)total_tiles * (blockIdx.x + 1)) / gridDim.x);

    if (warp == 0) {
        if (tid == 0) {
            uint32_t q = 0;
            const int tmask = (1 << p.tpi_shift) - 1;
            int z_next = 0;
            if (p.tpi_shift && tile_begin < tile_end) {
                const int img = tile_begin >> p.tpi_shift;
                z_next = p.rows ? (int)__ldg(p.rows + img) : img;
            }
            for (int tile = tile_begin; tile < tile_end; ++tile, ++q) {
                const uint32_t s = q % STAGES;
                const int z = z_next;
                if (p.tpi_shift && tile + 1 < tile_end) {
                    const int img = (tile + 1) >> p.tpi_shift;
                    z_next = p.rows ? (int)__ldg(p.rows + img) : img;
                }
                if (q >= (uint32_t)STAGES) mbar_wait(&empty_bar[s], ((q / STAGES) - 1) & 1);
                const uint32_t dst = smem_u32(sRing + (size_t)s * STAGE_BYTES);
                mbar_arrive_expect_tx(&full_bar[s], (uint32_t)STAGE_BYTES);
                if (p.tpi_shift) {
#pragma unroll
                    for (int c = 0; c < CPR; ++c) tma_load_3d(dst + c * IMG, &tmA, c * 64, (tile & tmask) * 128, z, &full_bar[s]);
                } else {
#pragma unroll
                    for (int c = 0; c < CPR; ++c) tma_load_2d(dst + c * IMG, &tmA, c * 64, tile * 128, &full_bar[s]);
                }
            }
        }
    } else if (warp >= 4) {
        const int wg = (warp - 4) >> 2, wt = tid & 127;
        float* st = sAcc + wg * 64 * LDA;
        const uint32_t w_base = smem_u32(sW);
        const int lr = wt & 63, half = wt >> 6;
        const int lrow = wg * 64 + lr;
        const uint32_t mW = (65536u + (uint32_t)p.Wp - 1u) / (uint32_t)p.Wp;
        const int tmask = (1 << p.tpi_shift) - 1;
        constexpr int NW = BN / 32;
        float d[BN / 2];
#pragma unroll
        for (int e = 0; e < BN / 2; ++e) d[e] = 0.f;
        for (int tile = tile_begin; tile < tile_end; ++tile) {
            const uint32_t q = (uint32_t)(tile - tile_begin), s = q % STAGES;
            const int64_t r = (int64_t)tile * 128 + lrow;
            int i = (int)(r / p.G);
            int rem = (int)(r - (int64_t)i * p.G);
            bool inside = r < p.M;
            if (p.tpi_shift) {
                i = tile >> p.tpi_shift;
                rem = ((tile & tmask) << 7) + lrow;
                inside = rem < p.G;
            }
            mbar_wait(&full_bar[s], (q / STAGES) & 1);
            wgmma_fence();
            const uint32_t win = smem_u32(sRing + (size_t)s * STAGE_BYTES) + (uint32_t)(wg * 64 * 128);
#pragma unroll
            for (int t = 0; t < NTAPS; ++t) {
#pragma unroll
                for (int c = 0; c < CPR; ++c) {
                    const uint64_t a = desc_kmajor(win + (uint32_t)(c * IMG) + (uint32_t)p.shift[t] * 128u);
                    const uint64_t b = desc_kmajor(w_base + (uint32_t)((t * CPR + c) * B_CHUNK));
#pragma unroll
                    for (int kk = 0; kk < 4; ++kk)
                        WgmmaBf16<BN, 0, 0>::mma(d, a + 2 * kk, b + 2 * kk, (t | c | kk) != 0 ? 1u : 0u);
                }
            }
            wgmma_commit();
            const int Y = (int)(((uint32_t)rem * mW) >> 16), X = rem - Y * p.Wp;
            const bool valid = inside && (Y < p.vH) && (X < p.vW);
            int64_t o1 = 0, ob = 0;
            if (p.out_mode == WOUT_S2D2) {
                const int64_t cell = ((int64_t)i * 10 + (Y >> 1)) * 10 + (X >> 1);
                const int cls = (Y & 1) * 2 + (X & 1);
                o1 = cell * 128 + cls * 32; ob = cell * 4 + cls;
            } else {
                ob = ((int64_t)i * 100 + Y * 10 + X) * 4;
            }
            uint32_t mb[NW];
#pragma unroll
            for (int g = 0; g < NW; ++g) mb[g] = 0xFFFFFFFFu;
            if (p.mask_bits != nullptr && valid) {
                if (NW == 4) {
                    const int4 t = ldg16(p.mask_bits + ob);
                    mb[0] = (uint32_t)t.x; mb[1 % NW] = (uint32_t)t.y; mb[2 % NW] = (uint32_t)t.z; mb[3 % NW] = (uint32_t)t.w;
                } else if (NW == 2) {
                    const uint2 t = __ldg(reinterpret_cast<const uint2*>(p.mask_bits + ob));
                    mb[0] = t.x; mb[1 % NW] = t.y;
                } else {
                    mb[0] = __ldg(p.mask_bits + ob);
                }
            }
            wgmma_wait<0>();
            wgmma_fence_operands(d);
            if ((tid & 31) == 0) mbar_arrive(&empty_bar[s]);
            named_bar(1 + wg, 128);
            stage_acc(st, LDA, wt, d);
            named_bar(1 + wg, 128);
#pragma unroll
            for (int g = 0; g < NW; ++g) {
                if ((g & 1) != half) continue;
                if (!valid || g * 32 >= p.N) continue;
                uint32_t v[32];
#pragma unroll
                for (int e = 0; e < 8; ++e) {
                    const float4 f = *reinterpret_cast<const float4*>(st + lr * LDA + g * 32 + 4 * e);
                    v[4 * e] = __float_as_uint(f.x); v[4 * e + 1] = __float_as_uint(f.y);
                    v[4 * e + 2] = __float_as_uint(f.z); v[4 * e + 3] = __float_as_uint(f.w);
                }
                if (p.bias) {
                    const float4* bp = reinterpret_cast<const float4*>(p.bias + g * 32);
#pragma unroll
                    for (int e = 0; e < 8; ++e) {
                        const float4 bv = __ldg(bp + e);
                        v[4 * e] = __float_as_uint(fmaf(__uint_as_float(v[4 * e]), p.scale, bv.x));
                        v[4 * e + 1] = __float_as_uint(fmaf(__uint_as_float(v[4 * e + 1]), p.scale, bv.y));
                        v[4 * e + 2] = __float_as_uint(fmaf(__uint_as_float(v[4 * e + 2]), p.scale, bv.z));
                        v[4 * e + 3] = __float_as_uint(fmaf(__uint_as_float(v[4 * e + 3]), p.scale, bv.w));
                    }
                } else {
#pragma unroll
                    for (int e = 0; e < 32; ++e) v[e] = __float_as_uint(__uint_as_float(v[e]) * p.scale);
                }
                if (p.relu) {
                    uint32_t bits = 0u;
#pragma unroll
                    for (int e = 0; e < 32; ++e) {
                        const float f = __uint_as_float(v[e]);
                        bits |= (f > 0.f ? 1u : 0u) << e;
                    }
                    if (p.mask_out) p.mask_out[ob + g] = bits;
                }
                if (p.mask_bits) {
#pragma unroll
                    for (int e = 0; e < 32; ++e) if (!((mb[g] >> e) & 1u)) v[e] = 0u;
                }
                int4 w[4];
                if (p.relu) {
#pragma unroll
                    for (int e = 0; e < 4; ++e) {
                        w[e].x = (int)pack_bf16x2_relu(__uint_as_float(v[8 * e]), __uint_as_float(v[8 * e + 1]));
                        w[e].y = (int)pack_bf16x2_relu(__uint_as_float(v[8 * e + 2]), __uint_as_float(v[8 * e + 3]));
                        w[e].z = (int)pack_bf16x2_relu(__uint_as_float(v[8 * e + 4]), __uint_as_float(v[8 * e + 5]));
                        w[e].w = (int)pack_bf16x2_relu(__uint_as_float(v[8 * e + 6]), __uint_as_float(v[8 * e + 7]));
                    }
                } else {
#pragma unroll
                for (int e = 0; e < 4; ++e) {
                    w[e].x = (int)pack_bf16x2(__uint_as_float(v[8 * e]), __uint_as_float(v[8 * e + 1]));
                    w[e].y = (int)pack_bf16x2(__uint_as_float(v[8 * e + 2]), __uint_as_float(v[8 * e + 3]));
                    w[e].z = (int)pack_bf16x2(__uint_as_float(v[8 * e + 4]), __uint_as_float(v[8 * e + 5]));
                    w[e].w = (int)pack_bf16x2(__uint_as_float(v[8 * e + 6]), __uint_as_float(v[8 * e + 7]));
                }
                }
                if (p.out_mode == WOUT_DACT1) {
                    int4* brow = reinterpret_cast<int4*>(st + lr * LDA) + 8 * g + 4 * (g & 1);
#pragma unroll
                    for (int e = 0; e < 4; ++e) brow[e] = w[e];
                } else {
                    bf16* dst = p.out + o1 + g * 32;
                    st_global_32b(dst, w[0], w[1]);
                    st_global_32b(dst + 16, w[2], w[3]);
                }
            }
            if (p.out_mode == WOUT_DACT1) {
                if (half == 0)
                    *reinterpret_cast<int64_t*>(st + lr * LDA + BN) = valid ? ((int64_t)i * 441 + 2 * Y * 21 + 2 * X) * 32 : -1;
                named_bar(1 + wg, 128);
#pragma unroll
                for (int m = 0; m < 8; ++m) {
                    const int k = m * 128 + wt, g = (k >> 2) & 3, e = k & 3;
                    const float* srow = st + (k >> 4) * LDA;
                    const int64_t o = *reinterpret_cast<const int64_t*>(srow + BN);
                    if (o < 0) continue;
                    const int4 val = reinterpret_cast<const int4*>(srow)[8 * g + 4 * (g & 1) + e];
                    *reinterpret_cast<int4*>(p.out + o + (g >> 1) * 21 * 32 + (g & 1) * 32 + e * 8) = val;
                }
            }
        }
    }
}

template <int BN, int CPR, int STAGES, int NTAPS>
static int launch_conv_win(const WinParams& p, cudaStream_t s, const char* what) {
    if (p.ntaps != NTAPS) return fail(B200RL_ERR_INVALID_ARGUMENT, "%s: %d taps, kernel instance has %d", what, p.ntaps, NTAPS);
    if (p.out_mode != WOUT_S2D2 && p.out_mode != WOUT_DACT1)
        return fail(B200RL_ERR_INVALID_ARGUMENT, "%s: dense and conv3 data-gradient outputs run on tc_conv_win_t", what);
    if (p.out_mode == WOUT_DACT1 && (BN != 128 || p.N != 128))
        return fail(B200RL_ERR_INVALID_ARGUMENT, "%s: the conv2 data gradient stores 4 groups of 32 channels per cell", what);
    const size_t smem = (size_t)p.ntaps * CPR * BN * 128 + (size_t)STAGES * p.WR * 128 * CPR + conv_win_acc_bytes<BN>() + 1024;
    static SmemAttrCache attr;
    if (int rc = attr.ensure(tc_conv_win<BN, CPR, STAGES, NTAPS>, smem, what)) return rc;
    if ((int64_t)p.G * p.Wp >= 65536 || p.G < 1 || p.N % 32 != 0)
        return fail(B200RL_ERR_INVALID_ARGUMENT, "%s: grid %d x width %d outside the epilogue's multiply-shift range, or N %% 32 != 0", what, p.G, p.Wp);
    if (p.rows && !p.tpi_shift) return fail(B200RL_ERR_INVALID_ARGUMENT, "%s: the image gather needs image-aligned tiling", what);
    if (p.tpi_shift && (128 << p.tpi_shift) < p.G) return fail(B200RL_ERR_INVALID_ARGUMENT, "%s: tiles per image too small", what);
    const int total = p.tpi_shift ? (int)((int64_t)p.n << p.tpi_shift) : (int)ceil_div(p.M, 128);
    int grid = num_sms();
    if (grid > total) grid = total;
    CUtensorMap tmA;
    memset(&tmA, 0, sizeof(tmA));
    int rc;
    if (p.tpi_shift) rc = make_tmap_3d(&tmA, p.A, p.n_images, p.G, (int64_t)CPR * 64, p.WR, what);
    else rc = make_tmap_2d(&tmA, p.A, p.M, (int64_t)CPR * 64, p.WR, what);
    if (rc) return rc;
    tc_conv_win<BN, CPR, STAGES, NTAPS><<<grid, kConvWinThreads, smem, s>>>(tmA, p, total);
    return check_launch(what);
}

constexpr int kConvWinTThreads = 384;
constexpr int kConvWinTLds = 64 + 4;
template <int BP>
__host__ __device__ constexpr size_t conv_win_t_stage_bytes() { return (size_t)2 * BP * kConvWinTLds * sizeof(float); }

template <int R>
__device__ __forceinline__ void stage_acc_transposed(float* st, int wg_tid, const float (&d)[R]) {
    const int co = ((wg_tid >> 5) << 4) + ((wg_tid & 31) >> 2), pos = (wg_tid & 3) * 2;
#pragma unroll
    for (int j = 0; j < R / 4; ++j) {
        float* p0 = st + (8 * j + pos) * kConvWinTLds + co;
        p0[0] = d[4 * j];
        p0[kConvWinTLds] = d[4 * j + 1];
        p0[8] = d[4 * j + 2];
        p0[kConvWinTLds + 8] = d[4 * j + 3];
    }
}

template <int BP, int CPR, int STAGES, int NTAPS>
__global__ void __launch_bounds__(kConvWinTThreads, 1) tc_conv_win_t(const __grid_constant__ CUtensorMap tmA, const WinParams p,
                                                                     int total_tiles) {
    static_assert(BP % 128 == 0, "one thread per position row of a 128-row slice");
    static_assert(STAGES % 2 == 0, "each consumer warpgroup owns every other stage");
    constexpr int RPT = BP / 128;
    constexpr int A_CHUNK = 64 * 128;
    constexpr int LDS = kConvWinTLds;
    extern __shared__ uint8_t smem_raw[];
    __shared__ uint64_t full_bar[STAGES], empty_bar[STAGES];
    uint8_t* smem = reinterpret_cast<uint8_t*>((reinterpret_cast<uintptr_t>(smem_raw) + 1023) & ~uintptr_t(1023));
    const int tid = threadIdx.x, warp = tid >> 5;
    const int nchunks = NTAPS * CPR;
    const int K = nchunks * 64;
    const int IMG = p.WR * 128;
    const int STAGE_BYTES = IMG * CPR;
    uint8_t* sW = smem;
    uint8_t* sRing = smem + (size_t)nchunks * A_CHUNK;
    float* sAcc = reinterpret_cast<float*>(sRing + (size_t)STAGES * STAGE_BYTES);

    if (tid == 0) {
        for (int s = 0; s < STAGES; ++s) { mbar_init(&full_bar[s], 1); mbar_init(&empty_bar[s], 4); }
        fence_barrier_init();
        tma_prefetch_desc(&tmA);
    }
    for (int idx = tid; idx < nchunks * 64 * 8; idx += blockDim.x) {
        const int c16 = idx & 7;
        const int t = idx >> 3;
        const int r = t & 63, j = t >> 6;
        int4 v = make_int4(0, 0, 0, 0);
        if (r < p.N) v = ldg16(p.Bw + (int64_t)r * K + j * 64 + c16 * 8);
        *reinterpret_cast<int4*>(sW + (size_t)j * A_CHUNK + img_off(r, c16)) = v;
    }
    fence_proxy_async_smem();
    __syncthreads();
    const int tile_begin = (int)(((int64_t)total_tiles * blockIdx.x) / gridDim.x);
    const int tile_end = (int)(((int64_t)total_tiles * (blockIdx.x + 1)) / gridDim.x);

    if (warp == 0) {
        if (tid == 0) {
            uint32_t q = 0;
            for (int tile = tile_begin; tile < tile_end; ++tile, ++q) {
                const uint32_t s = q % STAGES;
                if (q >= (uint32_t)STAGES) mbar_wait(&empty_bar[s], ((q / STAGES) - 1) & 1);
                const uint32_t dst = smem_u32(sRing + (size_t)s * STAGE_BYTES);
                mbar_arrive_expect_tx(&full_bar[s], (uint32_t)STAGE_BYTES);
#pragma unroll
                for (int c = 0; c < CPR; ++c) tma_load_2d(dst + c * IMG, &tmA, c * 64, tile * BP, &full_bar[s]);
            }
        }
    } else if (warp >= 4) {
        const int wg = (warp - 4) >> 2, wt = tid & 127;
        float* st = sAcc + wg * BP * LDS;
        const uint32_t w_base = smem_u32(sW);
        const uint32_t mW = (65536u + (uint32_t)p.Wp - 1u) / (uint32_t)p.Wp;
        constexpr int NW = 2;
        float d[BP / 2];
#pragma unroll
        for (int e = 0; e < BP / 2; ++e) d[e] = 0.f;
        for (int tile = tile_begin + wg; tile < tile_end; tile += 2) {
            const uint32_t q = (uint32_t)(tile - tile_begin), s = q % STAGES;
            mbar_wait(&full_bar[s], (q / STAGES) & 1);
            wgmma_fence();
            const uint32_t win = smem_u32(sRing + (size_t)s * STAGE_BYTES);
#pragma unroll
            for (int t = 0; t < NTAPS; ++t) {
#pragma unroll
                for (int c = 0; c < CPR; ++c) {
                    const uint64_t b = desc_kmajor(win + (uint32_t)(c * IMG) + (uint32_t)p.shift[t] * 128u);
                    const uint64_t a = desc_kmajor(w_base + (uint32_t)((t * CPR + c) * A_CHUNK));
#pragma unroll
                    for (int kk = 0; kk < 4; ++kk)
                        WgmmaBf16<BP, 0, 0>::mma(d, a + 2 * kk, b + 2 * kk, (t | c | kk) != 0 ? 1u : 0u);
                }
            }
            wgmma_commit();
            bool valid[RPT];
            int64_t o1[RPT], o2[RPT], ob[RPT];
            uint32_t mb[RPT][NW];
#pragma unroll
            for (int rr = 0; rr < RPT; ++rr) {
                const int64_t r = (int64_t)tile * BP + rr * 128 + wt;
                const int i = (int)(r / p.G);
                const int rem = (int)(r - (int64_t)i * p.G);
                const int Y = (int)(((uint32_t)rem * mW) >> 16), X = rem - Y * p.Wp;
                valid[rr] = r < p.M && (Y < p.vH) && (X < p.vW);
                o2[rr] = 0;
                if (p.out_mode == WOUT_DENSE) {
                    const int64_t orow = ((int64_t)i * p.vH + Y) * p.vW + X;
                    o1[rr] = orow * p.N; ob[rr] = orow * (p.N >> 5);
                } else {
                    o1[rr] = ((int64_t)i * 100 + Y * 10 + X) * 64;
                    o2[rr] = ((int64_t)i * 121 + (Y + 1) * 11 + (X + 1)) * 64;
                    ob[rr] = ((int64_t)i * 81 + Y * 9 + X) * 2;
                }
                mb[rr][0] = mb[rr][1] = 0xFFFFFFFFu;
                if (p.mask_bits != nullptr && valid[rr]) {
                    const uint2 t = __ldg(reinterpret_cast<const uint2*>(p.mask_bits + ob[rr]));
                    mb[rr][0] = t.x; mb[rr][1] = t.y;
                }
            }
            wgmma_wait<0>();
            wgmma_fence_operands(d);
            if ((tid & 31) == 0) mbar_arrive(&empty_bar[s]);
            named_bar(1 + wg, 128);
            stage_acc_transposed(st, wt, d);
            named_bar(1 + wg, 128);
#pragma unroll
            for (int rr = 0; rr < RPT; ++rr) {
                float* srow = st + (rr * 128 + wt) * LDS;
#pragma unroll
                for (int g = 0; g < NW; ++g) {
                    if (!valid[rr] || g * 32 >= p.N) continue;
                    uint32_t v[32];
#pragma unroll
                    for (int e = 0; e < 8; ++e) {
                        const float4 f = *reinterpret_cast<const float4*>(srow + g * 32 + 4 * e);
                        v[4 * e] = __float_as_uint(f.x); v[4 * e + 1] = __float_as_uint(f.y);
                        v[4 * e + 2] = __float_as_uint(f.z); v[4 * e + 3] = __float_as_uint(f.w);
                    }
                    if (p.bias) {
                        const float4* bp = reinterpret_cast<const float4*>(p.bias + g * 32);
#pragma unroll
                        for (int e = 0; e < 8; ++e) {
                            const float4 bv = __ldg(bp + e);
                            v[4 * e] = __float_as_uint(fmaf(__uint_as_float(v[4 * e]), p.scale, bv.x));
                            v[4 * e + 1] = __float_as_uint(fmaf(__uint_as_float(v[4 * e + 1]), p.scale, bv.y));
                            v[4 * e + 2] = __float_as_uint(fmaf(__uint_as_float(v[4 * e + 2]), p.scale, bv.z));
                            v[4 * e + 3] = __float_as_uint(fmaf(__uint_as_float(v[4 * e + 3]), p.scale, bv.w));
                        }
                    } else {
#pragma unroll
                        for (int e = 0; e < 32; ++e) v[e] = __float_as_uint(__uint_as_float(v[e]) * p.scale);
                    }
                    if (p.relu) {
                        uint32_t bits = 0u;
#pragma unroll
                        for (int e = 0; e < 32; ++e) bits |= (__uint_as_float(v[e]) > 0.f ? 1u : 0u) << e;
                        if (p.mask_out) p.mask_out[ob[rr] + g] = bits;
                    }
                    if (p.mask_bits) {
#pragma unroll
                        for (int e = 0; e < 32; ++e) if (!((mb[rr][g] >> e) & 1u)) v[e] = 0u;
                    }
                    int4 w[4];
                    if (p.relu) {
#pragma unroll
                        for (int e = 0; e < 4; ++e) {
                            w[e].x = (int)pack_bf16x2_relu(__uint_as_float(v[8 * e]), __uint_as_float(v[8 * e + 1]));
                            w[e].y = (int)pack_bf16x2_relu(__uint_as_float(v[8 * e + 2]), __uint_as_float(v[8 * e + 3]));
                            w[e].z = (int)pack_bf16x2_relu(__uint_as_float(v[8 * e + 4]), __uint_as_float(v[8 * e + 5]));
                            w[e].w = (int)pack_bf16x2_relu(__uint_as_float(v[8 * e + 6]), __uint_as_float(v[8 * e + 7]));
                        }
                    } else {
#pragma unroll
                        for (int e = 0; e < 4; ++e) {
                            w[e].x = (int)pack_bf16x2(__uint_as_float(v[8 * e]), __uint_as_float(v[8 * e + 1]));
                            w[e].y = (int)pack_bf16x2(__uint_as_float(v[8 * e + 2]), __uint_as_float(v[8 * e + 3]));
                            w[e].z = (int)pack_bf16x2(__uint_as_float(v[8 * e + 4]), __uint_as_float(v[8 * e + 5]));
                            w[e].w = (int)pack_bf16x2(__uint_as_float(v[8 * e + 6]), __uint_as_float(v[8 * e + 7]));
                        }
                    }
                    int4* brow = reinterpret_cast<int4*>(srow) + 4 * g;
#pragma unroll
                    for (int e = 0; e < 4; ++e) brow[e] = w[e];
                }
                *reinterpret_cast<longlong2*>(srow + 64) = make_longlong2(valid[rr] ? o1[rr] : -1, o2[rr]);
            }
            named_bar(1 + wg, 128);
#pragma unroll
            for (int m = 0; m < BP / 16; ++m) {
                const int k = m * 128 + wt, part = k & 7;
                const float* srow = st + (k >> 3) * LDS;
                const longlong2 off = *reinterpret_cast<const longlong2*>(srow + 64);
                if (off.x < 0) continue;
                const int4 val = reinterpret_cast<const int4*>(srow)[part];
                *reinterpret_cast<int4*>(p.out + off.x + part * 8) = val;
                if (p.out_mode == WOUT_DACT2) *reinterpret_cast<int4*>(p.out2 + off.y + part * 8) = val;
            }
        }
    }
}

template <int BP, int CPR, int STAGES, int NTAPS>
static int launch_conv_win_t(WinParams p, cudaStream_t s, const char* what) {
    if (p.ntaps != NTAPS) return fail(B200RL_ERR_INVALID_ARGUMENT, "%s: %d taps, kernel instance has %d", what, p.ntaps, NTAPS);
    if (p.N != 64) return fail(B200RL_ERR_INVALID_ARGUMENT, "%s: N = %d, the kernel computes 64 output channels", what, p.N);
    if ((int64_t)p.G * p.Wp >= 65536 || p.G < 1)
        return fail(B200RL_ERR_INVALID_ARGUMENT, "%s: grid %d x width %d outside the epilogue's multiply-shift range", what, p.G, p.Wp);
    if (p.rows || p.tpi_shift) return fail(B200RL_ERR_INVALID_ARGUMENT, "%s: the channel-major kernel walks a contiguous linear grid", what);
    if (p.out_mode != WOUT_DENSE && p.out_mode != WOUT_DACT2)
        return fail(B200RL_ERR_INVALID_ARGUMENT, "%s: only bf16 dense and conv3 data-gradient outputs in this kernel", what);
    int maxs = 0;
    for (int t = 0; t < NTAPS; ++t) maxs = p.shift[t] > maxs ? p.shift[t] : maxs;
    p.WR = (BP + maxs + 7) & ~7;
    if (p.WR > 256) return fail(B200RL_ERR_INVALID_ARGUMENT, "%s: window of %d rows exceeds a TMA box", what, p.WR);
    const size_t smem = (size_t)NTAPS * CPR * 64 * 128 + (size_t)STAGES * p.WR * 128 * CPR + conv_win_t_stage_bytes<BP>() + 1024;
    static SmemAttrCache attr;
    if (int rc = attr.ensure(tc_conv_win_t<BP, CPR, STAGES, NTAPS>, smem, what)) return rc;
    const int total = (int)ceil_div(p.M, BP);
    int grid = num_sms();
    if (grid > total) grid = total;
    CUtensorMap tmA;
    memset(&tmA, 0, sizeof(tmA));
    if (int rc = make_tmap_2d(&tmA, p.A, p.M, (int64_t)CPR * 64, p.WR, what)) return rc;
    tc_conv_win_t<BP, CPR, STAGES, NTAPS><<<grid, kConvWinTThreads, smem, s>>>(tmA, p, total);
    return check_launch(what);
}

}
```

Before: 1.196 million.

## Fuse u8 conv1 and conv2 forward into one warp-specialized kernel

Replaces the separate int8 conv1 kernel and the conv2 window kernel with a single kernel that computes conv1 per image into a double-buffered shared-memory act1 tile, then runs conv2 from that tile with weights resident in shared memory. This removes a kernel launch and part of the act1 round trip between conv1 and conv2 in the u8 observation path. The conv2 epilogue is factored into shared helpers, and the fused kernel uses register reallocation between producer and MMA warps. In exchange it takes a large shared-memory footprint and fewer pipeline stages, and adds more complex cross-warp synchronisation.

```diff
diff --git a/cleanrl_b200/csrc/net_tc.cu b/cleanrl_b200/csrc/net_tc.cu
--- a/cleanrl_b200/csrc/net_tc.cu
+++ b/cleanrl_b200/csrc/net_tc.cu
@@ -173,16 +173,22 @@
     return wide_dhead_bytes(n, L) + colsum_f32_ws(n, A1);
 }
 
+static void conv2_fwd_params(WinParams& wp, const NatureLayout& L, const NatureActs& Q, const float* params, const bf16* P, bf16* act,
+                             int64_t n) {
+    win_defaults(wp); win_conv2(wp, act + Q.act1, n);
+    wp.Bw = P + L.w2f; wp.N = 64; wp.vH = 9; wp.vW = 9; wp.out_mode = WOUT_DENSE; wp.out = act + Q.act2;
+    wp.bias = params + L.c2b; wp.relu = 1; wp.mask_out = reinterpret_cast<uint32_t*>(act + Q.m2);
+}
 static int trunk_fwd(const NatureLayout& L, const NatureActs& Q, const float* params, const bf16* P, bf16* act, int64_t n,
-                     cudaStream_t s) {
+                     bool conv2_fused, cudaStream_t s) {
     int rc;
     KGemmParams p;
     WinParams wp;
-    win_defaults(wp); win_conv2(wp, act + Q.act1, n);
-    wp.Bw = P + L.w2f; wp.N = 64; wp.vH = 9; wp.vW = 9; wp.out_mode = WOUT_DENSE; wp.out = act + Q.act2;
-    wp.bias = params + L.c2b; wp.relu = 1; wp.mask_out = reinterpret_cast<uint32_t*>(act + Q.m2);
-    { ProfScope ps(s, "conv2_fwd", 2.0 * n * 81 * 64 * 512, (double)n * ((12800 + 5184) * 2 + 648));
-      if ((rc = launch_conv_win_t<128, 2, 2, 4>(wp, s, "naturecnn/conv2"))) return rc; }
+    if (!conv2_fused) {
+        conv2_fwd_params(wp, L, Q, params, P, act, n);
+        ProfScope ps(s, "conv2_fwd", 2.0 * n * 81 * 64 * 512, (double)n * ((12800 + 5184) * 2 + 648));
+        if ((rc = launch_conv_win_t<128, 2, 2, 4>(wp, s, "naturecnn/conv2"))) return rc;
+    }
     win_defaults(wp); win_conv3(wp, act + Q.act2, n);
     wp.Bw = P + L.w3f; wp.N = 64; wp.vH = 7; wp.vW = 7; wp.out_mode = WOUT_DENSE; wp.out = act + Q.act3;
     wp.bias = params + L.c3b; wp.relu = 1; wp.mask_out = reinterpret_cast<uint32_t*>(act + Q.m3);
@@ -407,13 +413,15 @@
         x0 = act + Q.x0; x0rows = nullptr;
     }
     if (obs_format == B200RL_OBS_S2D_U8) {
-        Conv1U8Params cp;
+        Conv12U8Params cp;
         memset(&cp, 0, sizeof(cp));
         cp.rows = rows; cp.n = (int)n; cp.n_images = rows ? (int64_t)1 << 24 : n;
         cp.limbs = reinterpret_cast<const int8_t*>(P + L.w1l); cp.sc = reinterpret_cast<const float*>(P + L.w1sc);
-        cp.bias = params + L.c1b; cp.out = act + Q.act1; cp.mask_out = reinterpret_cast<uint32_t*>(act + Q.m1);
-        ProfScope ps(s, "conv1_fwd", 2.0 * n * 400 * 32 * 256, (double)n * (28224 + 12800 * 2 + 1600));
-        if ((rc = launch_conv1_i8(cp, obs, s, "naturecnn/conv1_i8"))) return rc;
+        cp.bias = params + L.c1b; cp.m1 = reinterpret_cast<uint32_t*>(act + Q.m1);
+        conv2_fwd_params(cp.c2, L, Q, params, P, act, n);
+        ProfScope ps(s, "conv12_fwd", 2.0 * n * 400 * 32 * 256 + 2.0 * n * 81 * 64 * 512,
+                     (double)n * (28224 + 12800 * 2 + 1600 + 5184 * 2 + 648));
+        if ((rc = launch_conv12_fwd_u8(cp, obs, act + Q.act1, s, "naturecnn/conv12_u8"))) return rc;
     } else {
     win_defaults(wp); win_conv1(wp, x0, x0rows, n);
     wp.Bw = P + L.w1f; wp.N = 32; wp.vH = 20; wp.vW = 20; wp.out_mode = WOUT_S2D2; wp.out = act + Q.act1;
@@ -421,7 +429,7 @@
     { ProfScope ps(s, "conv1_fwd", 2.0 * n * 400 * 32 * 256, (double)n * ((28224 + 12800) * 2 + 1600));
       if ((rc = launch_conv_win<32, 1, 9, 4>(wp, s, "naturecnn/conv1"))) return rc; }
     }
-    if ((rc = trunk_fwd(L, Q, params, P, act, n, s))) return rc;
+    if ((rc = trunk_fwd(L, Q, params, P, act, n, obs_format == B200RL_OBS_S2D_U8, s))) return rc;
     if (L.wide) {
         ProfScope ps(s, "heads_fwd", 2.0 * n * 512 * (A + 1), (double)n * (1024 + 4 * (A + 1)) + (double)L.G * 1024);
         return wide_head_fwd(L, P, act + Q.hid, n, A + 1, head_out, s);
@@ -612,7 +620,7 @@
         lstm::lstm_conv1_fwd<<<(unsigned)grid, lstm::kThreads, lstm::conv1_fwd_smem(), s>>>(cp);
         if ((rc = check_launch("lstm/conv1"))) return rc;
     }
-    if ((rc = trunk_fwd(L, Q.T, params, P, act, M, s))) return rc;
+    if ((rc = trunk_fwd(L, Q.T, params, P, act, M, false, s))) return rc;
     float* gx = reinterpret_cast<float*>(ab + Q.gx);
     { ProfScope ps(s, "lstm_ih_fwd", 2.0 * M * 512 * 512, (double)M * (1024 + 2048) + 512.0 * 1024);
       if ((rc = wide_head_fwd(L, P, act + Q.T.hid, M, 512, gx, s))) return rc; }
diff --git a/cleanrl_b200/csrc/tc_conv1_u8.cuh b/cleanrl_b200/csrc/tc_conv1_u8.cuh
--- a/cleanrl_b200/csrc/tc_conv1_u8.cuh
+++ b/cleanrl_b200/csrc/tc_conv1_u8.cuh
@@ -72,134 +72,6 @@
     if (idx == 0) {
         sc[co] = s / 128.0f / 255.0f;
         sc[32 + co] = s / 16384.0f / 255.0f;
-    }
-}
-
-struct Conv1U8Params {
-    const int64_t* rows;
-    int n;
-    int64_t n_images;
-    const int8_t* limbs;
-    const float* sc;
-    const float* bias;
-    bf16* out;
-    uint32_t* mask_out;
-};
-
-constexpr int kConv1I8Threads = 384;
-template <int STAGES>
-__global__ void __launch_bounds__(kConv1I8Threads, 1) tc_conv1_i8(const __grid_constant__ CUtensorMap tmA, const Conv1U8Params p, int total_tiles) {
-    constexpr int BN = 64, WR = 144, NTAPS = 4;
-    constexpr int STAGE_BYTES = WR * 128;
-    constexpr int B_CHUNK = BN * 64;
-    extern __shared__ uint8_t smem_raw[];
-    __shared__ uint64_t full_bar[STAGES], empty_bar[STAGES];
-    __shared__ __align__(16) float s_sc[32], s_bias[32];
-    uint8_t* smem = reinterpret_cast<uint8_t*>((reinterpret_cast<uintptr_t>(smem_raw) + 1023) & ~uintptr_t(1023));
-    const int tid = threadIdx.x, warp = tid >> 5;
-    uint8_t* sW = smem;
-    uint8_t* sRing = smem + NTAPS * B_CHUNK;
-
-    if (tid == 0) {
-        for (int s = 0; s < STAGES; ++s) { mbar_init(&full_bar[s], 1); mbar_init(&empty_bar[s], 8); }
-        fence_barrier_init();
-        tma_prefetch_desc(&tmA);
-    }
-    for (int idx = tid; idx < NTAPS * BN * 4; idx += blockDim.x) {
-        const int c16 = idx & 3;
-        const int t = (idx >> 2) & 3;
-        const int r = idx >> 4;
-        *reinterpret_cast<int4*>(sW + t * B_CHUNK + img64_off(r, c16)) = ldg16(p.limbs + r * 256 + t * 64 + c16 * 16);
-    }
-    if (tid < 32) { s_sc[tid] = p.sc[32 + tid]; s_bias[tid] = p.bias[tid]; }
-    fence_proxy_async_smem();
-    __syncthreads();
-    const int tile_begin = (int)(((int64_t)total_tiles * blockIdx.x) / gridDim.x);
-    const int tile_end = (int)(((int64_t)total_tiles * (blockIdx.x + 1)) / gridDim.x);
-
-    if (warp == 0) {
-        if (tid == 0) {
-            uint32_t q = 0;
-            int z_next = 0;
-            if (tile_begin < tile_end) {
-                const int img = tile_begin >> 1;
-                z_next = p.rows ? (int)__ldg(p.rows + img) : img;
-            }
-            for (int tile = tile_begin; tile < tile_end; ++tile, ++q) {
-                const uint32_t s = q % STAGES;
-                const int z = z_next;
-                if (tile + 1 < tile_end) {
-                    const int img = (tile + 1) >> 1;
-                    z_next = p.rows ? (int)__ldg(p.rows + img) : img;
-                }
-                if (q >= (uint32_t)STAGES) mbar_wait(&empty_bar[s], ((q / STAGES) - 1) & 1);
-                mbar_arrive_expect_tx(&full_bar[s], (uint32_t)STAGE_BYTES);
-                tma_load_3d(smem_u32(sRing + (size_t)s * STAGE_BYTES), &tmA, 0, (tile & 1) * 128, z, &full_bar[s]);
-            }
-        }
-    } else if (warp >= 4) {
-        const int wg = (warp - 4) >> 2, wt = tid & 127, lane = tid & 31, qd = lane & 3;
-        const uint32_t w_base = smem_u32(sW);
-        constexpr int off[4] = {0, 1, 21, 22};
-        int acc[2][32];
-#pragma unroll
-        for (int e = 0; e < 2; ++e)
-#pragma unroll
-            for (int c = 0; c < 32; ++c) acc[e][c] = 0;
-        for (int tile = tile_begin; tile < tile_end; ++tile) {
-            const uint32_t q = (uint32_t)(tile - tile_begin), s = q % STAGES;
-            mbar_wait(&full_bar[s], (q / STAGES) & 1);
-            wgmma_fence();
-            const uint32_t win = smem_u32(sRing + (size_t)s * STAGE_BYTES) + (uint32_t)(wg * 64 * 128);
-#pragma unroll
-            for (int e = 0; e < 2; ++e) {
-#pragma unroll
-                for (int t = 0; t < NTAPS; ++t) {
-                    const int po = e + off[t];
-                    const uint64_t a = desc_kmajor(win + (uint32_t)((po >> 1) * 128 + (po & 1) * 64));
-                    const uint64_t b = desc_kmajor_sw64(w_base + (uint32_t)(t * B_CHUNK));
-#pragma unroll
-                    for (int kk = 0; kk < 2; ++kk) wgmma_u8s8_n64(acc[e], a + 2 * kk, b + 2 * kk, (t | kk) != 0 ? 1u : 0u);
-                }
-            }
-            wgmma_commit();
-            wgmma_wait<0>();
-            wgmma_fence_operands(acc[0]);
-            wgmma_fence_operands(acc[1]);
-            if (lane == 0) mbar_arrive(&empty_bar[s]);
-            const int i = tile >> 1;
-#pragma unroll
-            for (int e = 0; e < 2; ++e) {
-#pragma unroll
-                for (int hr = 0; hr < 2; ++hr) {
-                    const int lrow = wg * 64 + ((wt >> 5) << 4) + (lane >> 2) + 8 * hr;
-                    const int rem = 2 * (((tile & 1) << 7) + lrow) + e;
-                    const int Y = (rem * 3121) >> 16, X = rem - Y * 21;
-                    const bool valid = rem < 441 && Y < 20 && X < 20;
-                    const int64_t cell = ((int64_t)i * 10 + (Y >> 1)) * 10 + (X >> 1);
-                    const int cls = (Y & 1) * 2 + (X & 1);
-                    uint32_t bits = 0u, pk[4];
-#pragma unroll
-                    for (int j = 0; j < 4; ++j) {
-                        const int co = 8 * j + 2 * qd;
-                        const float f0 = fmaf((float)(acc[e][4 * j + 2 * hr] * 128 + acc[e][4 * (j + 4) + 2 * hr]), s_sc[co], s_bias[co]);
-                        const float f1 = fmaf((float)(acc[e][4 * j + 2 * hr + 1] * 128 + acc[e][4 * (j + 4) + 2 * hr + 1]), s_sc[co + 1],
-                                              s_bias[co + 1]);
-                        bits |= (f0 > 0.f ? 1u : 0u) << co;
-                        bits |= (f1 > 0.f ? 1u : 0u) << (co + 1);
-                        pk[j] = pack_bf16x2_relu(f0, f1);
-                    }
-                    bits |= __shfl_xor_sync(0xffffffffu, bits, 1);
-                    bits |= __shfl_xor_sync(0xffffffffu, bits, 2);
-                    if (valid) {
-                        if (qd == 0) p.mask_out[cell * 4 + cls] = bits;
-                        uint32_t* dst = reinterpret_cast<uint32_t*>(reinterpret_cast<uint8_t*>(p.out) + (cell * 4 + cls) * 64);
-#pragma unroll
-                        for (int j = 0; j < 4; ++j) dst[4 * j + qd] = pk[j];
-                    }
-                }
-            }
-        }
     }
 }
 
@@ -496,20 +368,219 @@
     return check_launch(what);
 }
 
-constexpr int kConv1I8Stages = 8;
-static int launch_conv1_i8(const Conv1U8Params& p, const void* frames_rm, cudaStream_t s, const char* what) {
-    constexpr int STAGES = kConv1I8Stages;
-    const size_t smem = (size_t)4 * 64 * 64 + (size_t)STAGES * 144 * 128 + 1024;
-    const int total = p.n * 2;
+struct Conv12U8Params {
+    const int64_t* rows;
+    int n;
+    int64_t n_images;
+    const int8_t* limbs;
+    const float* sc;
+    const float* bias;
+    uint32_t* m1;
+    WinParams c2;
+};
+
+constexpr int kC12Threads = 512, kC12Stages = 4;
+constexpr int kC12StageBytes = 144 * 128;
+constexpr int kC12LimbChunk = 64 * 64;
+constexpr int kC12W2Chunk = 64 * 128;
+constexpr int kC12A1Rows = 144;
+constexpr int kC12A1Chunk = kC12A1Rows * 128, kC12A1Bytes = 2 * kC12A1Chunk;
+static_assert(conv_win_t_stage_bytes<128>() / 2 <= (size_t)kC12A1Bytes, "conv2's transpose tile reuses a consumed act1 image");
+constexpr int kC12RegsProducer = 40, kC12RegsMma = 152;
+static_assert(128 * kC12RegsProducer + 384 * kC12RegsMma <= 65536, "register budgets exceed the SM");
+static size_t conv12_fwd_smem() {
+    return (size_t)4 * kC12LimbChunk + (size_t)8 * kC12W2Chunk + 2 * (size_t)kC12A1Bytes + (size_t)kC12Stages * kC12StageBytes + 1024;
+}
+
+__global__ void __launch_bounds__(kC12Threads, 1) tc_conv12_fwd_u8(const __grid_constant__ CUtensorMap tmA, const __grid_constant__ CUtensorMap tmY,
+                                                                 const Conv12U8Params p) {
+    constexpr int STAGES = kC12Stages, NTAPS = 4;
+    extern __shared__ uint8_t smem_raw[];
+    __shared__ uint64_t full_bar[STAGES], empty_bar[STAGES], a1full[2], a1empty[2];
+    __shared__ __align__(16) float s_sc[32], s_bias[32];
+    uint8_t* smem = reinterpret_cast<uint8_t*>((reinterpret_cast<uintptr_t>(smem_raw) + 1023) & ~uintptr_t(1023));
+    uint8_t* sW1 = smem;
+    uint8_t* sW2 = sW1 + NTAPS * kC12LimbChunk;
+    uint8_t* sA1 = sW2 + 8 * kC12W2Chunk;
+    uint8_t* sRing = sA1 + 2 * kC12A1Bytes;
+    const int tid = threadIdx.x, warp = tid >> 5, lane = tid & 31;
+    if (tid == 0) {
+        for (int s = 0; s < STAGES; ++s) { mbar_init(&full_bar[s], 1); mbar_init(&empty_bar[s], 8); }
+        for (int b = 0; b < 2; ++b) { mbar_init(&a1full[b], 8); mbar_init(&a1empty[b], 4); }
+        fence_barrier_init();
+        tma_prefetch_desc(&tmA);
+        tma_prefetch_desc(&tmY);
+    }
+    for (int idx = tid; idx < NTAPS * 64 * 4; idx += blockDim.x) {
+        const int c16 = idx & 3;
+        const int t = (idx >> 2) & 3;
+        const int r = idx >> 4;
+        *reinterpret_cast<int4*>(sW1 + t * kC12LimbChunk + img64_off(r, c16)) = ldg16(p.limbs + r * 256 + t * 64 + c16 * 16);
+    }
+    for (int idx = tid; idx < 8 * 64 * 8; idx += blockDim.x) {
+        const int c16 = idx & 7, t = idx >> 3;
+        const int r = t & 63, j = t >> 6;
+        *reinterpret_cast<int4*>(sW2 + (size_t)j * kC12W2Chunk + img_off(r, c16)) = ldg16(p.c2.Bw + r * 512 + j * 64 + c16 * 8);
+    }
+    if (tid < 32) { s_sc[tid] = p.sc[32 + tid]; s_bias[tid] = p.bias[tid]; }
+    fence_proxy_async_smem();
+    __syncthreads();
+    const int img_begin = (int)(((int64_t)p.n * blockIdx.x) / gridDim.x);
+    const int img_end = (int)(((int64_t)p.n * (blockIdx.x + 1)) / gridDim.x);
+    const int tile_begin = 2 * img_begin, tile_end = 2 * img_end;
+
+    if (warp < 4) {
+        setmaxnreg_dec<kC12RegsProducer>();
+        if (tid == 0) {
+            uint32_t q = 0;
+            int z_next = 0;
+            if (tile_begin < tile_end) z_next = p.rows ? (int)__ldg(p.rows + img_begin) : img_begin;
+            for (int tile = tile_begin; tile < tile_end; ++tile, ++q) {
+                const uint32_t s = q % STAGES;
+                const int z = z_next;
+                if (tile + 1 < tile_end) {
+                    const int img = (tile + 1) >> 1;
+                    z_next = p.rows ? (int)__ldg(p.rows + img) : img;
+                }
+                if (q >= (uint32_t)STAGES) mbar_wait(&empty_bar[s], ((q / STAGES) - 1) & 1);
+                mbar_arrive_expect_tx(&full_bar[s], (uint32_t)kC12StageBytes);
+                tma_load_3d(smem_u32(sRing + (size_t)s * kC12StageBytes), &tmA, 0, (tile & 1) * 128, z, &full_bar[s]);
+            }
+        }
+    } else if (warp < 12) {
+        setmaxnreg_inc<kC12RegsMma>();
+        const int wg = (warp - 4) >> 2, wt = tid & 127, qd = lane & 3;
+        const uint32_t w_base = smem_u32(sW1);
+        constexpr int off[4] = {0, 1, 21, 22};
+        int acc[2][32];
+#pragma unroll
+        for (int e = 0; e < 2; ++e)
+#pragma unroll
+            for (int c = 0; c < 32; ++c) acc[e][c] = 0;
+        for (int tile = tile_begin; tile < tile_end; ++tile) {
+            const uint32_t q = (uint32_t)(tile - tile_begin), s = q % STAGES;
+            const int ji = (int)(q >> 1), buf = ji & 1;
+            mbar_wait(&full_bar[s], (q / STAGES) & 1);
+            wgmma_fence();
+            const uint32_t win = smem_u32(sRing + (size_t)s * kC12StageBytes) + (uint32_t)(wg * 64 * 128);
+#pragma unroll
+            for (int e = 0; e < 2; ++e) {
+#pragma unroll
+                for (int t = 0; t < NTAPS; ++t) {
+                    const int po = e + off[t];
+                    const uint64_t a = desc_kmajor(win + (uint32_t)((po >> 1) * 128 + (po & 1) * 64));
+                    const uint64_t b = desc_kmajor_sw64(w_base + (uint32_t)(t * kC12LimbChunk));
+#pragma unroll
+                    for (int kk = 0; kk < 2; ++kk) wgmma_u8s8_n64(acc[e], a + 2 * kk, b + 2 * kk, (t | kk) != 0 ? 1u : 0u);
+                }
+            }
+            wgmma_commit();
+            wgmma_wait<0>();
+            wgmma_fence_operands(acc[0]);
+            wgmma_fence_operands(acc[1]);
+            if (lane == 0) mbar_arrive(&empty_bar[s]);
+            if ((tile & 1) == 0 && ji >= 2) mbar_wait(&a1empty[buf], ((ji >> 1) - 1) & 1);
+            const uint32_t a1 = smem_u32(sA1 + (size_t)buf * kC12A1Bytes) + (uint32_t)(4 * qd);
+            const int i = tile >> 1;
+#pragma unroll
+            for (int e = 0; e < 2; ++e) {
+#pragma unroll
+                for (int hr = 0; hr < 2; ++hr) {
+                    const int lrow = wg * 64 + ((wt >> 5) << 4) + (lane >> 2) + 8 * hr;
+                    const int rem = 2 * (((tile & 1) << 7) + lrow) + e;
+                    const int Y = (rem * 3121) >> 16, X = rem - Y * 21;
+                    const bool valid = rem < 441 && Y < 20 && X < 20;
+                    const int cl = (Y >> 1) * 10 + (X >> 1);
+                    const int cls = (Y & 1) * 2 + (X & 1);
+                    uint32_t bits = 0u, pk[4];
+#pragma unroll
+                    for (int j = 0; j < 4; ++j) {
+                        const int co = 8 * j + 2 * qd;
+                        const float f0 = fmaf((float)(acc[e][4 * j + 2 * hr] * 128 + acc[e][4 * (j + 4) + 2 * hr]), s_sc[co], s_bias[co]);
+                        const float f1 = fmaf((float)(acc[e][4 * j + 2 * hr + 1] * 128 + acc[e][4 * (j + 4) + 2 * hr + 1]), s_sc[co + 1],
+                                              s_bias[co + 1]);
+                        bits |= (f0 > 0.f ? 1u : 0u) << co;
+                        bits |= (f1 > 0.f ? 1u : 0u) << (co + 1);
+                        pk[j] = pack_bf16x2_relu(f0, f1);
+                    }
+                    bits |= __shfl_xor_sync(0xffffffffu, bits, 1);
+                    bits |= __shfl_xor_sync(0xffffffffu, bits, 2);
+                    if (valid) {
+                        if (qd == 0) p.m1[((int64_t)i * 100 + cl) * 4 + cls] = bits;
+                        const uint32_t dst = a1 + (uint32_t)((cls >> 1) * kC12A1Chunk);
+#pragma unroll
+                        for (int j = 0; j < 4; ++j) sts32(dst + img_off(cl, 4 * (cls & 1) + j), pk[j]);
+                    }
+                }
+            }
+            if (tile & 1) {
+                fence_proxy_async_smem();
+                __syncwarp();
+                if (lane == 0) mbar_arrive(&a1full[buf]);
+            }
+        }
+    } else {
+        setmaxnreg_inc<kC12RegsMma>();
+        const int wt = tid - 384;
+        const uint32_t w_base = smem_u32(sW2);
+        const uint32_t mW = (65536u + (uint32_t)p.c2.Wp - 1u) / (uint32_t)p.c2.Wp;
+        float d[64];
+#pragma unroll
+        for (int e = 0; e < 64; ++e) d[e] = 0.f;
+        for (int ji = 0; ji < img_end - img_begin; ++ji) {
+            const int i = img_begin + ji, buf = ji & 1;
+            uint8_t* img = sA1 + (size_t)buf * kC12A1Bytes;
+            const uint32_t win = smem_u32(img);
+            mbar_wait(&a1full[buf], (ji >> 1) & 1);
+            if (wt == 0) {
+                tma_store_3d(&tmY, win, 0, 0, i);
+                tma_store_3d(&tmY, win + kC12A1Chunk, 64, 0, i);
+                bulk_commit();
+            }
+            wgmma_fence();
+#pragma unroll
+            for (int t = 0; t < 4; ++t) {
+#pragma unroll
+                for (int c = 0; c < 2; ++c) {
+                    const uint64_t b = desc_kmajor(win + (uint32_t)(c * kC12A1Chunk) + (uint32_t)p.c2.shift[t] * 128u);
+                    const uint64_t a = desc_kmajor(w_base + (uint32_t)((t * 2 + c) * kC12W2Chunk));
+#pragma unroll
+                    for (int kk = 0; kk < 4; ++kk) WgmmaBf16<128, 0, 0>::mma(d, a + 2 * kk, b + 2 * kk, (t | c | kk) != 0 ? 1u : 0u);
+                }
+            }
+            wgmma_commit();
+            WinTRow row[1];
+            row[0] = win_t_row(p.c2, (int64_t)i * 100 + wt, mW);
+            row[0].valid = row[0].valid && wt < 100;
+            wgmma_wait<0>();
+            wgmma_fence_operands(d);
+            if (wt == 0) bulk_wait_read<0>();
+            named_bar(1, 128);
+            win_t_epilogue<1>(p.c2, reinterpret_cast<float*>(img), wt, d, row, 1);
+            __syncwarp();
+            if (lane == 0) mbar_arrive(&a1empty[buf]);
+        }
+        if (wt == 0) bulk_wait<0>();
+    }
+}
+
+static int launch_conv12_fwd_u8(const Conv12U8Params& p, const void* frames_rm, bf16* act1, cudaStream_t s, const char* what) {
+    const WinParams& c2 = p.c2;
+    if (c2.N != 64 || c2.ntaps != 4 || c2.G != 100 || c2.Wp != 10 || c2.out_mode != WOUT_DENSE || c2.mask_bits)
+        return fail(B200RL_ERR_INVALID_ARGUMENT, "%s: conv2 must be the dense 2x2 window convolution of the 10x10 cells", what);
+    for (int t = 0; t < 4; ++t)
+        if (c2.shift[t] < 0 || c2.shift[t] > kC12A1Rows - 128) return fail(B200RL_ERR_INVALID_ARGUMENT, "%s: conv2 tap shift %d", what, c2.shift[t]);
+    const size_t smem = conv12_fwd_smem();
     int grid = num_sms();
-    if (grid > total) grid = total;
-    CUtensorMap tmA;
-    memset(&tmA, 0, sizeof(tmA));
-    int rc = make_tmap_pairs_u8(&tmA, frames_rm, p.n_images, what);
-    if (rc) return rc;
+    if (grid > p.n) grid = p.n;
+    CUtensorMap tmA, tmY;
+    memset(&tmA, 0, sizeof(tmA)); memset(&tmY, 0, sizeof(tmY));
+    int rc;
+    if ((rc = make_tmap_pairs_u8(&tmA, frames_rm, p.n_images, what))) return rc;
+    if ((rc = make_tmap_3d(&tmY, act1, p.n, 100, 128, 128, what))) return rc;
     static SmemAttrCache attr;
-    if ((rc = attr.ensure(tc_conv1_i8<STAGES>, smem, what))) return rc;
-    tc_conv1_i8<STAGES><<<grid, kConv1I8Threads, smem, s>>>(tmA, p, total);
+    if ((rc = attr.ensure(tc_conv12_fwd_u8, smem, what))) return rc;
+    tc_conv12_fwd_u8<<<grid, kC12Threads, smem, s>>>(tmA, tmY, p);
     return check_launch(what);
 }
 
diff --git a/cleanrl_b200/csrc/tc_conv_win.cuh b/cleanrl_b200/csrc/tc_conv_win.cuh
--- a/cleanrl_b200/csrc/tc_conv_win.cuh
+++ b/cleanrl_b200/csrc/tc_conv_win.cuh
@@ -291,6 +291,115 @@
     }
 }
 
+struct WinTRow {
+    bool valid;
+    int64_t o1, o2, ob;
+    uint32_t mb[2];
+};
+__device__ __forceinline__ WinTRow win_t_row(const WinParams& p, int64_t r, uint32_t mW) {
+    WinTRow w;
+    const int i = (int)(r / p.G);
+    const int rem = (int)(r - (int64_t)i * p.G);
+    const int Y = (int)(((uint32_t)rem * mW) >> 16), X = rem - Y * p.Wp;
+    w.valid = r < p.M && (Y < p.vH) && (X < p.vW);
+    w.o2 = 0;
+    if (p.out_mode == WOUT_DENSE) {
+        const int64_t orow = ((int64_t)i * p.vH + Y) * p.vW + X;
+        w.o1 = orow * p.N; w.ob = orow * (p.N >> 5);
+    } else {
+        w.o1 = ((int64_t)i * 100 + Y * 10 + X) * 64;
+        w.o2 = ((int64_t)i * 121 + (Y + 1) * 11 + (X + 1)) * 64;
+        w.ob = ((int64_t)i * 81 + Y * 9 + X) * 2;
+    }
+    w.mb[0] = w.mb[1] = 0xFFFFFFFFu;
+    if (p.mask_bits != nullptr && w.valid) {
+        const uint2 t = __ldg(reinterpret_cast<const uint2*>(p.mask_bits + w.ob));
+        w.mb[0] = t.x; w.mb[1] = t.y;
+    }
+    return w;
+}
+
+template <int RPT, int R>
+__device__ __forceinline__ void win_t_epilogue(const WinParams& p, float* st, int wt, const float (&d)[R], const WinTRow (&row)[RPT],
+                                               int bar) {
+    constexpr int LDS = kConvWinTLds;
+    constexpr int NW = 2;
+    stage_acc_transposed(st, wt, d);
+    named_bar(bar, 128);
+#pragma unroll
+    for (int rr = 0; rr < RPT; ++rr) {
+        float* srow = st + (rr * 128 + wt) * LDS;
+#pragma unroll
+        for (int g = 0; g < NW; ++g) {
+            if (!row[rr].valid || g * 32 >= p.N) continue;
+            uint32_t v[32];
+#pragma unroll
+            for (int e = 0; e < 8; ++e) {
+                const float4 f = *reinterpret_cast<const float4*>(srow + g * 32 + 4 * e);
+                v[4 * e] = __float_as_uint(f.x); v[4 * e + 1] = __float_as_uint(f.y);
+                v[4 * e + 2] = __float_as_uint(f.z); v[4 * e + 3] = __float_as_uint(f.w);
+            }
+            if (p.bias) {
+                const float4* bp = reinterpret_cast<const float4*>(p.bias + g * 32);
+#pragma unroll
+                for (int e = 0; e < 8; ++e) {
+                    const float4 bv = __ldg(bp + e);
+                    v[4 * e] = __float_as_uint(fmaf(__uint_as_float(v[4 * e]), p.scale, bv.x));
+                    v[4 * e + 1] = __float_as_uint(fmaf(__uint_as_float(v[4 * e + 1]), p.scale, bv.y));
+                    v[4 * e + 2] = __float_as_uint(fmaf(__uint_as_float(v[4 * e + 2]), p.scale, bv.z));
+                    v[4 * e + 3] = __float_as_uint(fmaf(__uint_as_float(v[4 * e + 3]), p.scale, bv.w));
+                }
+            } else {
+#pragma unroll
+                for (int e = 0; e < 32; ++e) v[e] = __float_as_uint(__uint_as_float(v[e]) * p.scale);
+            }
+            if (p.relu) {
+                uint32_t bits = 0u;
+#pragma unroll
+                for (int e = 0; e < 32; ++e) bits |= (__uint_as_float(v[e]) > 0.f ? 1u : 0u) << e;
+                if (p.mask_out) p.mask_out[row[rr].ob + g] = bits;
+            }
+            if (p.mask_bits) {
+#pragma unroll
+                for (int e = 0; e < 32; ++e) if (!((row[rr].mb[g] >> e) & 1u)) v[e] = 0u;
+            }
+            int4 w[4];
+            if (p.relu) {
+#pragma unroll
+                for (int e = 0; e < 4; ++e) {
+                    w[e].x = (int)pack_bf16x2_relu(__uint_as_float(v[8 * e]), __uint_as_float(v[8 * e + 1]));
+                    w[e].y = (int)pack_bf16x2_relu(__uint_as_float(v[8 * e + 2]), __uint_as_float(v[8 * e + 3]));
+                    w[e].z = (int)pack_bf16x2_relu(__uint_as_float(v[8 * e + 4]), __uint_as_float(v[8 * e + 5]));
+                    w[e].w = (int)pack_bf16x2_relu(__uint_as_float(v[8 * e + 6]), __uint_as_float(v[8 * e + 7]));
+                }
+            } else {
+#pragma unroll
+                for (int e = 0; e < 4; ++e) {
+                    w[e].x = (int)pack_bf16x2(__uint_as_float(v[8 * e]), __uint_as_float(v[8 * e + 1]));
+                    w[e].y = (int)pack_bf16x2(__uint_as_float(v[8 * e + 2]), __uint_as_float(v[8 * e + 3]));
+                    w[e].z = (int)pack_bf16x2(__uint_as_float(v[8 * e + 4]), __uint_as_float(v[8 * e + 5]));
+                    w[e].w = (int)pack_bf16x2(__uint_as_float(v[8 * e + 6]), __uint_as_float(v[8 * e + 7]));
+                }
+            }
+            int4* brow = reinterpret_cast<int4*>(srow) + 4 * g;
+#pragma unroll
+            for (int e = 0; e < 4; ++e) brow[e] = w[e];
+        }
+        *reinterpret_cast<longlong2*>(srow + 64) = make_longlong2(row[rr].valid ? row[rr].o1 : -1, row[rr].o2);
+    }
+    named_bar(bar, 128);
+#pragma unroll
+    for (int m = 0; m < RPT * 8; ++m) {
+        const int k = m * 128 + wt, part = k & 7;
+        const float* srow = st + (k >> 3) * LDS;
+        const longlong2 off = *reinterpret_cast<const longlong2*>(srow + 64);
+        if (off.x < 0) continue;
+        const int4 val = reinterpret_cast<const int4*>(srow)[part];
+        *reinterpret_cast<int4*>(p.out + off.x + part * 8) = val;
+        if (p.out_mode == WOUT_DACT2) *reinterpret_cast<int4*>(p.out2 + off.y + part * 8) = val;
+    }
+}
+
 template <int BP, int CPR, int STAGES, int NTAPS>
 __global__ void __launch_bounds__(kConvWinTThreads, 1) tc_conv_win_t(const __grid_constant__ CUtensorMap tmA, const WinParams p,
                                                                      int total_tiles) {
@@ -346,7 +455,6 @@
         float* st = sAcc + wg * BP * LDS;
         const uint32_t w_base = smem_u32(sW);
         const uint32_t mW = (65536u + (uint32_t)p.Wp - 1u) / (uint32_t)p.Wp;
-        constexpr int NW = 2;
         float d[BP / 2];
 #pragma unroll
         for (int e = 0; e < BP / 2; ++e) d[e] = 0.f;
@@ -367,109 +475,14 @@
                 }
             }
             wgmma_commit();
-            bool valid[RPT];
-            int64_t o1[RPT], o2[RPT], ob[RPT];
-            uint32_t mb[RPT][NW];
-#pragma unroll
-            for (int rr = 0; rr < RPT; ++rr) {
-                const int64_t r = (int64_t)tile * BP + rr * 128 + wt;
-                const int i = (int)(r / p.G);
-                const int rem = (int)(r - (int64_t)i * p.G);
-                const int Y = (int)(((uint32_t)rem * mW) >> 16), X = rem - Y * p.Wp;
-                valid[rr] = r < p.M && (Y < p.vH) && (X < p.vW);
-                o2[rr] = 0;
-                if (p.out_mode == WOUT_DENSE) {
-                    const int64_t orow = ((int64_t)i * p.vH + Y) * p.vW + X;
-                    o1[rr] = orow * p.N; ob[rr] = orow * (p.N >> 5);
-                } else {
-                    o1[rr] = ((int64_t)i * 100 + Y * 10 + X) * 64;
-                    o2[rr] = ((int64_t)i * 121 + (Y + 1) * 11 + (X + 1)) * 64;
-                    ob[rr] = ((int64_t)i * 81 + Y * 9 + X) * 2;
-                }
-                mb[rr][0] = mb[rr][1] = 0xFFFFFFFFu;
-                if (p.mask_bits != nullptr && valid[rr]) {
-                    const uint2 t = __ldg(reinterpret_cast<const uint2*>(p.mask_bits + ob[rr]));
-                    mb[rr][0] = t.x; mb[rr][1] = t.y;
-                }
-            }
+            WinTRow row[RPT];
+#pragma unroll
+            for (int rr = 0; rr < RPT; ++rr) row[rr] = win_t_row(p, (int64_t)tile * BP + rr * 128 + wt, mW);
             wgmma_wait<0>();
             wgmma_fence_operands(d);
             if ((tid & 31) == 0) mbar_arrive(&empty_bar[s]);
             named_bar(1 + wg, 128);
-            stage_acc_transposed(st, wt, d);
-            named_bar(1 + wg, 128);
-#pragma unroll
-            for (int rr = 0; rr < RPT; ++rr) {
-                float* srow = st + (rr * 128 + wt) * LDS;
-#pragma unroll
-                for (int g = 0; g < NW; ++g) {
-                    if (!valid[rr] || g * 32 >= p.N) continue;
-                    uint32_t v[32];
-#pragma unroll
-                    for (int e = 0; e < 8; ++e) {
-                        const float4 f = *reinterpret_cast<const float4*>(srow + g * 32 + 4 * e);
-                        v[4 * e] = __float_as_uint(f.x); v[4 * e + 1] = __float_as_uint(f.y);
-                        v[4 * e + 2] = __float_as_uint(f.z); v[4 * e + 3] = __float_as_uint(f.w);
-                    }
-                    if (p.bias) {
-                        const float4* bp = reinterpret_cast<const float4*>(p.bias + g * 32);
-#pragma unroll
-                        for (int e = 0; e < 8; ++e) {
-                            const float4 bv = __ldg(bp + e);
-                            v[4 * e] = __float_as_uint(fmaf(__uint_as_float(v[4 * e]), p.scale, bv.x));
-                            v[4 * e + 1] = __float_as_uint(fmaf(__uint_as_float(v[4 * e + 1]), p.scale, bv.y));
-                            v[4 * e + 2] = __float_as_uint(fmaf(__uint_as_float(v[4 * e + 2]), p.scale, bv.z));
-                            v[4 * e + 3] = __float_as_uint(fmaf(__uint_as_float(v[4 * e + 3]), p.scale, bv.w));
-                        }
-                    } else {
-#pragma unroll
-                        for (int e = 0; e < 32; ++e) v[e] = __float_as_uint(__uint_as_float(v[e]) * p.scale);
-                    }
-                    if (p.relu) {
-                        uint32_t bits = 0u;
-#pragma unroll
-                        for (int e = 0; e < 32; ++e) bits |= (__uint_as_float(v[e]) > 0.f ? 1u : 0u) << e;
-                        if (p.mask_out) p.mask_out[ob[rr] + g] = bits;
-                    }
-                    if (p.mask_bits) {
-#pragma unroll
-                        for (int e = 0; e < 32; ++e) if (!((mb[rr][g] >> e) & 1u)) v[e] = 0u;
-                    }
-                    int4 w[4];
-                    if (p.relu) {
-#pragma unroll
-                        for (int e = 0; e < 4; ++e) {
-                            w[e].x = (int)pack_bf16x2_relu(__uint_as_float(v[8 * e]), __uint_as_float(v[8 * e + 1]));
-                            w[e].y = (int)pack_bf16x2_relu(__uint_as_float(v[8 * e + 2]), __uint_as_float(v[8 * e + 3]));
-                            w[e].z = (int)pack_bf16x2_relu(__uint_as_float(v[8 * e + 4]), __uint_as_float(v[8 * e + 5]));
-                            w[e].w = (int)pack_bf16x2_relu(__uint_as_float(v[8 * e + 6]), __uint_as_float(v[8 * e + 7]));
-                        }
-                    } else {
-#pragma unroll
-                        for (int e = 0; e < 4; ++e) {
-                            w[e].x = (int)pack_bf16x2(__uint_as_float(v[8 * e]), __uint_as_float(v[8 * e + 1]));
-                            w[e].y = (int)pack_bf16x2(__uint_as_float(v[8 * e + 2]), __uint_as_float(v[8 * e + 3]));
-                            w[e].z = (int)pack_bf16x2(__uint_as_float(v[8 * e + 4]), __uint_as_float(v[8 * e + 5]));
-                            w[e].w = (int)pack_bf16x2(__uint_as_float(v[8 * e + 6]), __uint_as_float(v[8 * e + 7]));
-                        }
-                    }
-                    int4* brow = reinterpret_cast<int4*>(srow) + 4 * g;
-#pragma unroll
-                    for (int e = 0; e < 4; ++e) brow[e] = w[e];
-                }
-                *reinterpret_cast<longlong2*>(srow + 64) = make_longlong2(valid[rr] ? o1[rr] : -1, o2[rr]);
-            }
-            named_bar(1 + wg, 128);
-#pragma unroll
-            for (int m = 0; m < BP / 16; ++m) {
-                const int k = m * 128 + wt, part = k & 7;
-                const float* srow = st + (k >> 3) * LDS;
-                const longlong2 off = *reinterpret_cast<const longlong2*>(srow + 64);
-                if (off.x < 0) continue;
-                const int4 val = reinterpret_cast<const int4*>(srow)[part];
-                *reinterpret_cast<int4*>(p.out + off.x + part * 8) = val;
-                if (p.out_mode == WOUT_DACT2) *reinterpret_cast<int4*>(p.out2 + off.y + part * 8) = val;
-            }
+            win_t_epilogue<RPT>(p, st, wt, d, row, 1 + wg);
         }
     }
 }
```

Result: faster. 1.221 million, median of 6 (+2.0%).
